# hall-lab/svtyper

Hardware: AMD Instinct MI355X
Metric: breakpoints genotyped/sec (higher is better)
Workload: dtype f64

## Files before the change

svtyper_amd/csrc/svt_batch_create.h:

```cpp

struct StageTimer {
    bool on = std::getenv("SVT_TRACE") != nullptr;
    std::chrono::steady_clock::time_point t0 = std::chrono::steady_clock::now();
    void mark(const char* what)
    {
        if (!on) return;
        const auto t1 = std::chrono::steady_clock::now();
        std::fprintf(stderr, "[svt] %-28s %8.2f ms\n", what, std::chrono::duration<double, std::milli>(t1 - t0).count());
        t0 = t1;
    }
};

int record_error(uint32_t err_bits)
{
    return fail(SVT_ERR_INVALID, record_error_text(err_bits));
}

int check_stream_errors(svt_batch* b)
{
    if (b->layout != kLayoutStream || !b->d_err) return SVT_OK;
    uint32_t bits = 0;
    HIP_TRY(hipMemcpyAsync(&bits, b->d_err, sizeof(uint32_t), hipMemcpyDeviceToHost, b->stream));
    HIP_TRY(hipStreamSynchronize(b->stream));
    return bits ? record_error(bits) : SVT_OK;
}

int ensure_result_slots(svt_batch* b, uint64_t slots)
{
    const uint64_t bytes = std::max<uint64_t>(slots, 1) * ((b->flags & SVT_FLAG_RESULT96) ? sizeof(svt_result96) : sizeof(svt_result));
    if (bytes <= b->cap_out) return SVT_OK;
    HIP_TRY(hipStreamSynchronize(b->stream));
    const bool bound = b->out_dev != b->d_out;
    g_pool.put(b->device, b->d_out, b->cap_out);
    b->d_out = nullptr;
    b->cap_out = 0;
    void* p = nullptr;
    SVT_TRY(g_pool.get(b->device, bytes, &p, &b->cap_out));
    b->d_out = static_cast<svt_result*>(p);
    if (!bound) {
        b->out_dev = b->d_out;
        b->sargs.out = b->d_out;
        b->pargs.out = b->d_out;
    }
    return SVT_OK;
}

uint64_t max_batch_records()
{
    static const uint64_t cached = [] {
        uint64_t v = 0xFFFFFFF0ull - 1;
        if (const char* e = std::getenv("SVT_MAX_BATCH_RECORDS")) {
            const uint64_t w = std::strtoull(e, nullptr, 10);
            if (w > 0 && w < v) v = w;
        }
        return v;
    }();
    return cached;
}

SmallRegion small_region(size_t tab, const size_t region_bytes, const bool l10_in_front, const size_t l10_bytes = 0, const uint32_t n_l10 = 0)
{
    SmallRegion r;
    if (l10_in_front && tab + l10_bytes + region_bytes <= (160 * 1024 / 2)) {
        r.l10_where = kL10Shared;
        r.lds_l10 = (uint32_t)tab;
        r.l10_entries = n_l10;
        tab += l10_bytes;
    }
    if (tab + region_bytes <= 160 * 1024) {
        r.region = (uint32_t)tab;
        r.lds_bytes = tab + region_bytes;
    }
    return r;
}

int create_stream(const svt_evidence_batch* in, svt_batch* b, void* d_records_resident = nullptr, uint64_t resident_cap = 0,
                  bool defer_records = false)
{
    const uint64_t n = in->n_units;
    const uint64_t n_rec = n ? in->rec_offset[n] : 0;
    StageTimer tm;
    if (n_rec > max_batch_records())
        return fail(SVT_ERR_INVALID, "too many records in one batch (< 2^32): cut it with svt_chunk_bounds, or hand it to svt_genotype, which does");
    uint64_t max_f = 0;
    bool wide_var_length = false, all_hinted = n > 0;
    {
        const uint64_t kChunk = 16384, n_chunks = (n + kChunk - 1) / kChunk;
        struct Part { uint64_t max_f = 0; int bad = 0; bool wide = false, hinted = true; };
        std::vector<Part> parts(std::max<uint64_t>(n_chunks, 1));
        parallel_for(n_chunks, [&](uint64_t ch) {
            Part p;
            for (uint64_t u = ch * kChunk; u < std::min(n, (ch + 1) * kChunk); ++u) {
                if (in->rec_offset[u + 1] < in->rec_offset[u]) { p.bad |= 1; continue; }
                const uint64_t f = in->rec_offset[u + 1] - in->rec_offset[u];
                if (f > 0x3FFFFFFFull) p.bad |= 2;
                const svt_unit& U = in->units[u];
                if (U.svtype > SVT_SVTYPE_BND) p.bad |= 4;
                if ((U.libs >> 24) != 0 || (U.flags & ~SVT_UNIT_SKIP)) p.bad |= 8;
                const uint32_t w_lo = SVT_UNIT_LIBS_FIRST(U.libs), w_cnt = SVT_UNIT_LIBS_COUNT(U.libs);
                if (w_cnt && w_lo + w_cnt > in->n_libs) p.bad |= 16;
                p.hinted = p.hinted && w_cnt != 0;
                if (U.var_length < -(1 << 30) || U.var_length > (1 << 30)) p.wide = true;
                p.max_f = std::max(p.max_f, f);
            }
            parts[ch] = p;
        });
        int bad = 0;
        for (uint64_t ch = 0; ch < n_chunks; ++ch) {
            bad |= parts[ch].bad;
            max_f = std::max(max_f, parts[ch].max_f);
            wide_var_length = wide_var_length || parts[ch].wide;
            all_hinted = all_hinted && parts[ch].hinted;
        }
        if (bad & 1) return fail(SVT_ERR_INVALID, "rec_offset not monotone");
        if (bad & 2) return fail(SVT_ERR_INVALID, "unit with too many records");
        if (bad & 4) return fail(SVT_ERR_INVALID, "bad svtype");
        if (bad & 8) return fail(SVT_ERR_INVALID, "unit reserved/flags bits must be 0");
        if (bad & 16) return fail(SVT_ERR_INVALID, "unit library window beyond n_libs");
    }
    tm.mark("validate units");
    HostTables T;
    SVT_TRY(build_tables(in, max_f, T));
    if (wide_var_length) T.fast_geometry = false;

    b->window_tiles = (SVT_STREAM_R == 1 && SVT_WINDOW_TILES == 2 && n >= kTwoTilesMinUnits) ? 2 : SVT_STREAM_R;
#ifndef SVT_WINDOW_SPLIT
#define SVT_WINDOW_SPLIT 0
#endif
    const bool split_kinds = SVT_WINDOW_SPLIT && b->window_tiles == 2 && !(b->flags & SVT_FLAG_SSO_ASSOCIATION) && !std::getenv("SVT_NO_WINDOW_SPLIT");
    auto window_budget_kernel = [&]() { return split_kinds ? window_kernel_of_kind(2) : stream_kernel_of(b, b->window_tiles); };
    const uint32_t kUnitsPerWg = (uint32_t)kBlock * (uint32_t)b->window_tiles;
    std::vector<uint32_t> perm;
    std::vector<uint2> chunks;
    std::vector<WgDesc> windows;
    struct Group { uint32_t begin, end; WgDesc w; };
    std::vector<Group> groups;
    uint32_t max_win_bins = 0, max_win_libs = 0;
    uint64_t all_bins = 0;
    for (const LibDesc& L : T.libs) all_bins += L.n_bins + 1;
    const bool whole_batch_window = !all_hinted && n > 0 && in->n_libs <= 255 &&
                                    kSBins + all_bins * 4 + in->n_libs * sizeof(WinLib) + 64 + kWavesPerBlock * kStreamRingBytes <= (160 * 1024 / 2);
    const uint32_t whole_key = SVT_UNIT_LIBS(0u, in->n_libs);
    const bool may_window = in->n_libs > 1 && T.fast_geometry && !(b->flags & SVT_FLAG_GENERAL_TABLES);
    bool windowed = may_window && (all_hinted || whole_batch_window);
    const bool derive_windows = may_window && !windowed && n > 0 && T.narrow_bins;
    if (derive_windows) defer_records = false;
    b->records_resident = !defer_records;
    auto group_units = [&](auto&& hint_of) -> bool {
        std::vector<uint32_t> start(65537, 0u);
        std::vector<uint16_t> count_of(65536, 0);
        for (uint64_t u = 0; u < n; ++u) {
            const uint32_t h = hint_of(u), first = SVT_UNIT_LIBS_FIRST(h), cnt = SVT_UNIT_LIBS_COUNT(h);
            if (cnt == 0) return false;
            count_of[first] = std::max(count_of[first], (uint16_t)cnt);
            ++start[first + 1];
        }
        for (uint32_t k = 0; k < 65536u; ++k) start[k + 1] += start[k];
        perm.resize(n);
        groups.clear();
        {
            std::vector<uint32_t> at(start.begin(), start.end() - 1);
            for (uint64_t u = 0; u < n; ++u) perm[at[SVT_UNIT_LIBS_FIRST(hint_of(u))]++] = (uint32_t)u;
        }
        for (uint32_t k = 0; k < 65536u; ++k) {
            if (start[k + 1] == start[k]) continue;
            const uint32_t lo = k, cnt = count_of[k];
            WgDesc w{};
            w.lib_lo = lo;
            w.lib_cnt = cnt;
            w.bin_lo = T.libs[lo].tab_off;
            w.bin_cnt = T.libs[lo + cnt - 1].tab_off + T.libs[lo + cnt - 1].n_bins + 1 - w.bin_lo;
            max_win_bins = std::max(max_win_bins, w.bin_cnt);
            max_win_libs = std::max(max_win_libs, w.lib_cnt);
            groups.push_back(Group{start[k], start[k + 1], w});
        }
        return true;
    };
    auto cut_chunks = [&](const uint32_t per_chunk) {
        chunks.clear();
        windows.clear();
        for (const Group& g : groups) {
            const uint32_t units = g.end - g.begin, pieces = (units + per_chunk - 1) / per_chunk;
            for (uint32_t i = 0; i < pieces; ++i) {
                const uint32_t p0 = g.begin + (uint32_t)((uint64_t)units * i / pieces), p1 = g.begin + (uint32_t)((uint64_t)units * (i + 1) / pieces);
                chunks.push_back(make_uint2(p0, p1 - p0));
                windows.push_back(g.w);
            }
        }
    };
    if (windowed) {
        windowed = group_units([&](uint64_t u) -> uint32_t { return all_hinted ? in->units[u].libs : whole_key; });
        tm.mark("group units by library window");
    }
    const uint32_t n_l10 = (uint32_t)T.l10.size();
    T.l10.resize(((size_t)n_l10 + 127) / 128 * 128, 0.0);
    tm.mark("build tables");

    SVT_TRY(g_handles.get_stream(&b->stream));
    SVT_TRY(g_handles.get_event(&b->ev0, true));
    SVT_TRY(g_handles.get_event(&b->ev1, true));

    const uint64_t n_blk = std::max<uint64_t>((n_rec + kBlockRecords - 1) / kBlockRecords, 1);
    {
        Stager st(b->stream);
        void* p = nullptr;
        if (d_records_resident) {
            if (resident_cap < n_blk * 128) return fail(SVT_ERR_INTERNAL, "resident record buffer too small");
            b->d_records = d_records_resident;
            b->cap_records = resident_cap;
        } else {
            SVT_TRY(g_pool.get(b->device, n_blk * 128, &p, &b->cap_records, true));
            b->d_records = p;
        }
        if (n_blk * 128 > n_rec * 16)
            HIP_TRY(hipMemsetAsync(static_cast<char*>(b->d_records) + n_rec * 16, 0, n_blk * 128 - n_rec * 16, b->stream));
        if (!d_records_resident && !defer_records) SVT_TRY(st.copy(b->d_records, in->records, n_rec * sizeof(uint4)));
        SVT_TRY(g_pool.get(b->device, (n + 1) * sizeof(uint64_t), &p, &b->cap_off));
        b->d_off = static_cast<uint64_t*>(p);
        if (n) SVT_TRY(st.copy(b->d_off, in->rec_offset, (n + 1) * sizeof(uint64_t)));
        SVT_TRY(g_pool.get(b->device, std::max<uint64_t>(n, 1) * sizeof(svt_unit), &p, &b->cap_units));
        b->d_units = static_cast<svt_unit*>(p);
        SVT_TRY(st.copy(b->d_units, in->units, n * sizeof(svt_unit)));
        SVT_TRY(upload(&b->d_libs, T.libs, st));
        SVT_TRY(upload(&b->d_pm, T.pm, st));
        SVT_TRY(upload(&b->d_l10, T.l10, st));
        SVT_TRY(upload(&b->d_bins, T.bins, st));
        SVT_TRY(upload(&b->d_wtab, T.wtab, st));
        SVT_TRY(g_pool.get(b->device, std::max<uint64_t>(n, 1) * sizeof(svt_result), &p, &b->cap_out));
        b->d_out = static_cast<svt_result*>(p);
        SVT_TRY(g_handles.get_small(sizeof(uint32_t), &p));
        b->d_err = static_cast<uint32_t*>(p);
        HIP_TRY(hipMemsetAsync(b->d_err, 0, sizeof(uint32_t), b->stream));
        SVT_TRY(st.finish());
    }
    tm.mark("H2D CSR + tables (staged)");

    if (derive_windows) {
        void* pp = nullptr;
        SVT_TRY(g_pool.get(b->device, n * sizeof(uint32_t), &pp, &b->cap_perm));
        b->d_perm = static_cast<uint32_t*>(pp);
        const uint32_t n32 = (uint32_t)n;
        const unsigned waves = (unsigned)std::min<uint64_t>(n, 256ull * 32);
        const dim3 grid((waves + kScanBlock / kWave - 1) / (kScanBlock / kWave)), block(kScanBlock);
        hipLaunchKernelGGL(svt_window_scan_kernel, grid, block, 0, b->stream, static_cast<const uint4*>(b->d_records), b->d_off, n32, b->d_perm);
        HIP_TRY(hipGetLastError());
        std::vector<uint32_t> seen(n);
        HIP_TRY(hipMemcpyAsync(seen.data(), b->d_perm, n * sizeof(uint32_t), hipMemcpyDeviceToHost, b->stream));
        HIP_TRY(hipStreamSynchronize(b->stream));
        tm.mark("library windows from the records (device scan)");
        bool all_seen = true;
        for (uint64_t u = 0; u < n && all_seen; ++u) all_seen = seen[u] != 0u && SVT_UNIT_LIBS_FIRST(seen[u]) + SVT_UNIT_LIBS_COUNT(seen[u]) <= in->n_libs;
        if (all_seen) {
            windowed = group_units([&](uint64_t u) -> uint32_t { return seen[u]; });
            tm.mark("group units by library window");
        }
    }

    size_t kStreamLdsPerWg = (160 * 1024 / 3) & ~size_t(127);
    constexpr size_t kStreamLdsPerWg2 = (160 * 1024 / 2) & ~size_t(127);
    constexpr size_t kLdsBin = 2 * sizeof(uint16_t);
    const size_t single_lds = kSBins + T.bins.size() * kLdsBin;
    const bool single = in->n_libs == 1 && T.fast_geometry && T.narrow_bins && single_lds + kWavesPerBlock * kStreamRingBytes <= 96 * 1024 &&
                        !(b->flags & SVT_FLAG_GENERAL_TABLES);
    const size_t window_lds = kSBins + (((size_t)max_win_bins * kLdsBin + 15) & ~size_t(15)) + (size_t)max_win_libs * sizeof(WinLib);
    windowed = windowed && T.narrow_bins && max_win_libs <= 32 && window_lds + kWavesPerBlock * kStreamRingBytes <= kStreamLdsPerWg2;
    b->mode = single ? kSingleLds : windowed ? kMultiLds : kGeneral;
    if (b->mode == kGeneral && in->n_libs > 1024)
        return fail(SVT_ERR_UNSUPPORTED, "more than 1024 libraries in a batch without usable library windows (svt_unit.libs)");
    bool identity = true;
    if (windowed) {
        uint32_t per_chunk = kUnitsPerWg;
        {
            int wgs = 3;
            hipFuncAttributes fa{};
            if (hipFuncGetAttributes(&fa, window_budget_kernel()) == hipSuccess && fa.numRegs > 0) wgs = std::max(1, std::min(8, 512 / ((fa.numRegs + 7) / 8 * 8)));
            else (void)hipGetLastError();
            const size_t lds = ((window_lds + 127) & ~size_t(127)) + kWavesPerBlock * kStreamRingBytes;
            const uint32_t resident = (uint32_t)std::min<size_t>((size_t)wgs, (160 * 1024) / lds) * cu_count(b->device);
            uint64_t n_min = 0;
            for (const Group& g : groups) n_min += (g.end - g.begin + kUnitsPerWg - 1) / kUnitsPerWg;
            per_chunk = balanced_units_per_wg(n, n_min, kUnitsPerWg, resident);
            if (per_chunk < kUnitsPerWg && resident) {
                const uint64_t rounds = (n_min + resident - 1) / resident;
                auto count = [&](uint32_t per) { uint64_t c = 0; for (const Group& g : groups) c += (g.end - g.begin + per - 1) / per; return c; };
                while (per_chunk < kUnitsPerWg && count(per_chunk) > rounds * resident) ++per_chunk;
            }
        }
        cut_chunks(per_chunk);
        Stager st(b->stream);
        void* pp = nullptr;
        for (uint64_t u = 0; u < n && identity; ++u) identity = perm[u] == (uint32_t)u;
        if (!identity) {
            if (!b->d_perm) {
                SVT_TRY(g_pool.get(b->device, std::max<uint64_t>(n, 1) * sizeof(uint32_t), &pp, &b->cap_perm));
                b->d_perm = static_cast<uint32_t*>(pp);
            }
            SVT_TRY(st.copy(b->d_perm, perm.data(), n * sizeof(uint32_t)));
        }
        SVT_TRY(upload(&b->d_chunks, chunks, st));
        SVT_TRY(upload(&b->d_windows, windows, st));
        SVT_TRY(st.finish());
        b->n_chunks = (uint32_t)chunks.size();
        uint32_t n_one = 0;
        while (n_one < b->n_chunks && windows[n_one].lib_cnt == 1u) ++n_one;
        bool ordered = true;
        for (uint32_t i = n_one; i < b->n_chunks && ordered; ++i) ordered = windows[i].lib_cnt != 1u;
        b->n_chunks_one = n_one;
        b->split_window_kinds = split_kinds && ordered;
    }
    if (b->d_perm && (!windowed || identity)) {
        g_pool.put(b->device, b->d_perm, b->cap_perm);
        b->d_perm = nullptr;
        b->cap_perm = 0;
    }
    StreamArgs& a = b->sargs;
    a.records = static_cast<const uint4*>(b->d_records);
    a.rec_offset = b->d_off;
    a.units = b->d_units;
    a.pm = b->d_pm;
    a.l10 = b->d_l10;
    a.libs = b->d_libs;
    a.bins = b->d_bins;
    a.wtab = b->d_wtab;
    a.n_l10 = n_l10;
    a.n_libs = in->n_libs;
    a.total_bins = (uint32_t)T.bins.size();
    a.last_blk = (uint32_t)(n_blk - 1);
    a.lds_bins = single ? a.total_bins : windowed ? max_win_bins : 0u;
    a.lds_libs = single || windowed ? 0u : in->n_libs;
    a.perm = b->d_perm;
    a.chunks = b->d_chunks;
    a.windows = b->d_windows;
    a.lds_winlibs = (uint32_t)(kSBins + (((size_t)a.lds_bins * kLdsBin + 15) & ~size_t(15)));
    size_t tables = a.lds_winlibs + (size_t)a.lds_libs * sizeof(LibDesc) + (windowed ? (size_t)max_win_libs * sizeof(WinLib) : 0);
    tables = (tables + 127) & ~size_t(127);
    if (single) {
        int wgs = 3;
        hipFuncAttributes fa{};
        if (hipFuncGetAttributes(&fa, stream_kernel_of(b, 1)) == hipSuccess && fa.numRegs > 0) wgs = std::max(1, std::min(8, 512 / ((fa.numRegs + 7) / 8 * 8)));
        else (void)hipGetLastError();
        const size_t by_lds = (160 * 1024) / (tables + kWavesPerBlock * kStreamRingBytes);
        b->one_tile_round_units = (uint64_t)std::min<size_t>((size_t)wgs, std::max<size_t>(by_lds, 1)) * cu_count(b->device) * kBlock;
    }
    {
        int wgs = 3;
        hipFuncAttributes fa{};
        if (hipFuncGetAttributes(&fa, b->mode == kMultiLds ? window_budget_kernel() : stream_kernel_of(b, tiles_per_wave(b, n))) == hipSuccess && fa.numRegs > 0)
            wgs = std::max(1, std::min(8, 512 / ((fa.numRegs + 7) / 8 * 8)));
        else
            (void)hipGetLastError();
        if (const char* e = std::getenv("SVT_STREAM_WGS_PER_CU")) wgs = std::max(1, std::atoi(e));
#ifdef SVT_FORCE_WGS
        wgs = SVT_FORCE_WGS;
#endif
        kStreamLdsPerWg = (160 * 1024 / (size_t)wgs) & ~size_t(127);
        b->wgs_per_cu = wgs;
    }
    const size_t l10_bytes = ((size_t)n_l10 * 8 + 127) & ~size_t(127);
    const size_t base_lds = tables + kWavesPerBlock * kStreamRingBytes;
    const size_t fit = std::max<size_t>(1, std::min<size_t>((size_t)b->wgs_per_cu, (160 * 1024) / base_lds));
    const size_t budget = ((160 * 1024) / fit) & ~size_t(127);
    (void)kStreamLdsPerWg;
    if (base_lds + l10_bytes <= budget) {
        a.l10_where = kL10Shared;
        a.lds_l10 = (uint32_t)tables;
        a.l10_lds_entries = n_l10;
        tables += l10_bytes;
    } else if (kStreamDepth == 1 && SVT_L10_THROUGH_RING) {
        a.l10_where = kL10Ring;
        a.l10_lds_entries = (uint32_t)std::min<uint64_t>((n_l10 + 127u) / 128u * 128u, kStreamRingBytes / 8);
    } else {
        a.l10_where = kL10Global;
        a.l10_lds_entries = 0;
    }
    a.lds_rings = (uint32_t)tables;
    if (b->mode == kSingleLds && a.l10_where != kL10Ring) {
        const size_t tab = (a.lds_winlibs + 127) & ~size_t(127);
        b->coop = small_region(tab, kCoopRegionBytes, true, l10_bytes, n_l10);
        if (b->coop.lds_bytes) {
            int wgs = 2;
            hipFuncAttributes fa{};
            if (hipFuncGetAttributes(&fa, coop_kernel_of(b)) == hipSuccess && fa.numRegs > 0) wgs = std::max(1, std::min(4, 512 / ((fa.numRegs + 7) / 8 * 8) * 4 / kCoopWaves));
            else (void)hipGetLastError();
            b->coop_resident = (uint32_t)std::min<size_t>((size_t)wgs, (160 * 1024) / b->coop.lds_bytes) * cu_count(b->device);
            if (b->coop.lds_bytes > 64 * 1024) HIP_TRY(hipFuncSetAttribute(coop_kernel_of(b), hipFuncAttributeMaxDynamicSharedMemorySize, (int)b->coop.lds_bytes));
        }
        b->split = small_region(tab, kSplitRegionBytes, true, l10_bytes, n_l10);
        if (b->split.lds_bytes > 64 * 1024)
            for (int lanes = 2; lanes <= 4; lanes += 2)
                HIP_TRY(hipFuncSetAttribute(split_kernel_of(b, lanes), hipFuncAttributeMaxDynamicSharedMemorySize, (int)b->split.lds_bytes));
    }
    if (b->mode == kMultiLds && a.l10_where != kL10Ring) {
        b->split = small_region((tables + 127) & ~size_t(127), kSplitRegionBytes, false);
        if (b->split.lds_bytes) {
            b->split.l10_where = a.l10_where;
            b->split.lds_l10 = a.lds_l10;
            b->split.l10_entries = a.l10_lds_entries;
        }
        if (b->split.lds_bytes > 64 * 1024)
            for (int lanes = 2; lanes <= 4; lanes += 2)
                if (lanes == 4 || !(b->flags & SVT_FLAG_SSO_ASSOCIATION))
                    HIP_TRY(hipFuncSetAttribute(split_kernel_of(b, lanes), hipFuncAttributeMaxDynamicSharedMemorySize, (int)b->split.lds_bytes));
    }
    a.n_units = n;
    a.unit_begin = 0;
    a.unit_end = (uint32_t)n;
    a.units_per_wg = (uint32_t)kBlock * (uint32_t)tiles_per_wave(b, n);
    a.result96 = (b->flags & SVT_FLAG_RESULT96) ? 1u : 0u;
    a.slot_begin = 0;
    b->resident_wgs = (uint32_t)std::min<size_t>((size_t)b->wgs_per_cu, (160 * 1024) / (tables + kWavesPerBlock * kStreamRingBytes)) *
                      cu_count(b->device);
    b->out_dev = b->d_out;
    b->out_slots = !a.result96 ? n : b->mode == kMultiLds ? (uint64_t)b->n_chunks * kBlock * (uint64_t)b->window_tiles : slots_of_launch(b, n);
    SVT_TRY(ensure_result_slots(b, b->out_slots));
    a.out = b->d_out;
    a.err = b->d_err;
    a.lib0 = T.libs[0];
    fill_gt_consts(a.c, in->split_weight, in->disc_weight);
    b->out_dev = b->d_out;
    b->lds_bytes = tables + kWavesPerBlock * kStreamRingBytes;
    if (b->lds_bytes > 160 * 1024) return fail(SVT_ERR_INVALID, "LDS budget exceeded");
    if (tm.on)
        std::fprintf(stderr, "[svt] kernel budget: %d workgroups/CU by registers, LDS %zu B/workgroup (%zu fit), log10 table (%u entries) %s (%u entries)\n",
                     b->wgs_per_cu, b->lds_bytes, (size_t)(160 * 1024) / std::max<size_t>(b->lds_bytes, 1), n_l10,
                     a.l10_where == kL10Shared ? "in LDS" : a.l10_where == kL10Ring ? "through the ring" : "through L2", a.l10_lds_entries);
    if (b->lds_bytes > 64 * 1024)
        for (int tiles = 1; tiles <= 2; ++tiles)
            if (b->mode != kGeneral || tiles == 1)
                HIP_TRY(hipFuncSetAttribute(stream_kernel_of(b, tiles), hipFuncAttributeMaxDynamicSharedMemorySize, (int)b->lds_bytes));
    if (b->lds_bytes > 64 * 1024 && b->split_window_kinds)
        for (int kind = 1; kind <= 2; ++kind)
            HIP_TRY(hipFuncSetAttribute(window_kernel_of_kind(kind), hipFuncAttributeMaxDynamicSharedMemorySize, (int)b->lds_bytes));
    return SVT_OK;
}
```

svtyper_amd/csrc/svt_batch_state.h:

```cpp


void free_batch(svt_batch* b)
{
    if (!b) return;
    (void)hipSetDevice(b->device);
    if (b->stream) (void)hipStreamSynchronize(b->stream);
    auto F = [](void* p) { g_handles.put_small(p); };
    g_pool.put(b->device, b->d_out, b->cap_out);
    g_pool.put(b->device, b->d_records, b->cap_records);
    g_pool.put(b->device, b->d_off, b->cap_off);
    g_pool.put(b->device, b->d_units, b->cap_units);
    g_pool.put(b->device, b->d_soff, b->cap_soff);
    g_pool.put(b->device, b->d_perm, b->cap_perm);
    F(b->d_chunks); F(b->d_windows);
    F(b->d_err);
    F(b->d_pm); F(b->d_l10); F(b->d_libs);
    F(b->d_bins); F(b->d_wtab);
    g_handles.put_event(b->ev0, true);
    g_handles.put_event(b->ev1, true);
    g_handles.put_stream(b->stream);
    delete b;
}

struct BatchFree {
    void operator()(svt_batch* b) const { free_batch(b); }
};
using BatchOwner = std::unique_ptr<svt_batch, BatchFree>;

int new_batch(BatchOwner* owner, int device, unsigned flags, int layout, uint64_t n_units, uint64_t n_records)
{
    owner->reset(new (std::nothrow) svt_batch());
    svt_batch* b = owner->get();
    if (!b) return fail(SVT_ERR_NOMEM, "out of host memory");
    b->device = device;
    b->flags = flags;
    b->layout = layout;
    b->n_units = n_units;
    b->n_records = n_records;
    return SVT_OK;
}

int check_device(int device)
{
    const int ndev = svt_device_count();
    if (ndev <= 0) return fail(SVT_ERR_NO_DEVICE, "no HIP device available (this library has no CPU fallback)");
    if (device < 0 || device >= ndev) return fail(SVT_ERR_NO_DEVICE, "device index out of range");
    return SVT_OK;
}

int select_device(int device)
{
    SVT_TRY(check_device(device));
    HIP_TRY(hipSetDevice(device));
    return SVT_OK;
}

const char* evidence_error(const svt_evidence_batch* in, unsigned flags, bool records_may_be_null = false)
{
    const uint64_t n = in->n_units;
    if (flags & ~kKnownFlags) return "unknown flag bits";
    if (n >= 0xFFFFFFF0ull) return "too many units in one batch (< 2^32)";
    if (in->n_libs == 0 || in->n_libs > 65536 || !in->libs) return "n_libs must be 1..65536";
    if (n && (!in->rec_offset || !in->units)) return "null unit arrays";
    if (n && in->rec_offset[0] != 0) return "rec_offset[0] must be 0";
    if (n && in->rec_offset[n] && !in->records && !records_may_be_null) return "null records";
    if (!(in->split_weight >= 0.0) || !(in->disc_weight >= 0.0) || !std::isfinite(in->split_weight) || !std::isfinite(in->disc_weight))
        return "weights must be finite and >= 0";
    return nullptr;
}

struct DevScratch {
    void* p = nullptr;
    ~DevScratch() { if (p) (void)hipFree(p); }
    int alloc(size_t bytes)
    {
        HIP_TRY(hipMalloc(&p, std::max<size_t>(bytes, 16)));
        return SVT_OK;
    }
    template <typename T> T* as() const { return static_cast<T*>(p); }
};

struct Pooled {
    int device;
    void* p = nullptr;
    uint64_t cap = 0;
    ~Pooled() { g_pool.put(device, p, cap); }
    int get(uint64_t bytes, bool records = false) { return g_pool.get(device, bytes, &p, &cap, records); }
    void* release() { void* q = p; p = nullptr; return q; }
};

struct CallStream {
    hipStream_t s = nullptr;
    ~CallStream() { if (s) g_handles.put_stream(s); }
    int take() { return g_handles.get_stream(&s); }
    void drain() { if (s) (void)hipStreamSynchronize(s); }
};

template <typename T>
int upload(T** dptr, const std::vector<T>& v, Stager& st)
{
    void* p = nullptr;
    const uint64_t bytes = std::max<size_t>(v.size(), 1) * sizeof(T);
    if (bytes <= (1u << 20)) SVT_TRY(g_handles.get_small(bytes, &p));
    else HIP_TRY(hipMalloc(&p, bytes));
    *dptr = static_cast<T*>(p);
    return st.copy(*dptr, v.data(), v.size() * sizeof(T));
}

template <typename T>
int upload(DevScratch& d, const std::vector<T>& v, Stager& st)
{
    SVT_TRY(d.alloc(v.size() * sizeof(T)));
    return st.copy(d.p, v.data(), v.size() * sizeof(T));
}

template <bool SSO>
const void* stream_kernel_for(int mode, int tiles)
{
    if (mode == kSingleLds && tiles == 2) return reinterpret_cast<const void*>(&svt_stream_kernel<SSO, kSingleLds, 2>);
    if (mode == kMultiLds && tiles == 2) return reinterpret_cast<const void*>(&svt_stream_kernel<SSO, kMultiLds, 2>);
    return mode == kSingleLds  ? reinterpret_cast<const void*>(&svt_stream_kernel<SSO, kSingleLds, SVT_STREAM_R>)
           : mode == kMultiLds ? reinterpret_cast<const void*>(&svt_stream_kernel<SSO, kMultiLds, SVT_STREAM_R>)
                               : reinterpret_cast<const void*>(&svt_stream_kernel<SSO, kGeneral, SVT_STREAM_R>);
}

const void* window_kernel_of_kind(int kind)
{
    return kind == 1 ? reinterpret_cast<const void*>(&svt_stream_kernel<false, kMultiLds, 2, 1>)
                     : reinterpret_cast<const void*>(&svt_stream_kernel<false, kMultiLds, 2, 2>);
}

const void* stream_kernel_of(const svt_batch* b, int tiles = SVT_STREAM_R)
{
    return (b->flags & SVT_FLAG_SSO_ASSOCIATION) ? stream_kernel_for<true>(b->mode, tiles) : stream_kernel_for<false>(b->mode, tiles);
}

const void* coop_kernel_of(const svt_batch* b)
{
    return (b->flags & SVT_FLAG_SSO_ASSOCIATION) ? reinterpret_cast<const void*>(&svt_coop_kernel<true, kSingleLds>)
                                                  : reinterpret_cast<const void*>(&svt_coop_kernel<false, kSingleLds>);
}

const void* split_kernel_of(const svt_batch* b, int lanes)
{
    const bool sso = (b->flags & SVT_FLAG_SSO_ASSOCIATION) != 0;
    if (b->mode == kMultiLds) {
        if (lanes == 2) return reinterpret_cast<const void*>(&svt_split_kernel<false, kMultiLds, 2>);
        return sso ? reinterpret_cast<const void*>(&svt_split_kernel<true, kMultiLds, 4>) : reinterpret_cast<const void*>(&svt_split_kernel<false, kMultiLds, 4>);
    }
    if (lanes == 2) return sso ? reinterpret_cast<const void*>(&svt_split_kernel<true, kSingleLds, 2>) : reinterpret_cast<const void*>(&svt_split_kernel<false, kSingleLds, 2>);
    return sso ? reinterpret_cast<const void*>(&svt_split_kernel<true, kSingleLds, 4>) : reinterpret_cast<const void*>(&svt_split_kernel<false, kSingleLds, 4>);
}

constexpr uint64_t kTwoTilesMinUnits = 768ull * kBlock * 9 / 8;
int tiles_per_wave(const svt_batch* b, uint64_t units)
{
#if SVT_STREAM_R == 1 && !defined(SVT_STREAM_ONE_TILE)
    if (b->mode == kSingleLds && units > (b->one_tile_round_units ? b->one_tile_round_units : kTwoTilesMinUnits)) return 2;
#endif
    (void)b; (void)units;
    return SVT_STREAM_R;
}

#ifndef SVT_L10_THROUGH_RING
#define SVT_L10_THROUGH_RING 0
#endif

inline uint32_t cu_count(int device)
{
    static std::mutex lock;
    static std::vector<int> known;
    std::lock_guard<std::mutex> g(lock);
    if ((size_t)device >= known.size()) known.resize((size_t)device + 1, 0);
    if (known[(size_t)device] == 0) {
        int v = 0;
        if (hipDeviceGetAttribute(&v, hipDeviceAttributeMultiprocessorCount, device) != hipSuccess || v <= 0) { (void)hipGetLastError(); v = 256; }
        known[(size_t)device] = v;
    }
    return (uint32_t)known[(size_t)device];
}

#ifndef SVT_WG_BALANCE
#define SVT_WG_BALANCE 1
#endif
#ifndef SVT_WG_MIN_FILL
#define SVT_WG_MIN_FILL 50
#endif
struct WgPlan { int tiles; uint32_t per_wg, n_wg; bool coop; int split; };
static std::atomic<int> g_wg_balance{SVT_WG_BALANCE && !std::getenv("SVT_NO_WG_BALANCE") ? SVT_WG_MIN_FILL : 0};
extern "C" int svt_debug_wg_balance(int min_fill_percent) { return g_wg_balance.exchange(std::max(0, std::min(100, min_fill_percent))); }
inline uint32_t balanced_units_per_wg(uint64_t units, uint64_t n_min, uint32_t full, uint32_t resident)
{
    const int min_fill = g_wg_balance.load(std::memory_order_relaxed);
    if (!min_fill || !resident || n_min <= resident) return full;
    const uint64_t rounds = (n_min + resident - 1) / resident;
    const uint64_t want = (units + rounds * resident - 1) / (rounds * resident);
    return want * 100 >= (uint64_t)full * (uint64_t)min_fill ? (uint32_t)want : full;
}
static std::atomic<uint32_t> g_force_per_wg{0}, g_force_tiles{0};
extern "C" void svt_debug_force_wg(uint32_t per_wg, uint32_t tiles) { g_force_per_wg = per_wg; g_force_tiles = tiles; }
#ifndef SVT_COOP_MAX_UNITS
#define SVT_COOP_MAX_UNITS (1ull << 40)
#endif
static std::atomic<uint64_t> g_coop_max_units{std::getenv("SVT_NO_COOP") ? uint64_t(0) : uint64_t(SVT_COOP_MAX_UNITS)};
static std::atomic<uint32_t> g_coop_per_wg{0};
extern "C" void svt_debug_coop(uint64_t max_units, uint32_t per_wg) { g_coop_max_units = max_units; g_coop_per_wg = per_wg; }
#ifndef SVT_SMALL_KIND
#define SVT_SMALL_KIND 0
#endif
#ifndef SVT_SPLIT4_CU_UNITS
#define SVT_SPLIT4_CU_UNITS 256
#endif
#ifndef SVT_SPLIT2_CU_UNITS
#define SVT_SPLIT2_CU_UNITS 512
#endif
#ifndef SVT_COOP_CU_UNITS
#define SVT_COOP_CU_UNITS 64
#endif
static std::atomic<int> g_small_kind{SVT_SMALL_KIND};
extern "C" int svt_debug_small_kind(int kind) { return g_small_kind.exchange(kind); }
int split_lanes_for(const svt_batch* b, uint64_t units)
{
    const int kind = g_small_kind.load(std::memory_order_relaxed);
    const bool sso = (b->flags & SVT_FLAG_SSO_ASSOCIATION) != 0;
    if (!b->split.lds_bytes || !units) return 0;
    if (kind == 3) return sso && b->mode == kMultiLds ? 0 : 2;
    if (kind == 4) return 4;
    if (kind != 0) return 0;
    const uint64_t cus = cu_count(b->device);
    const bool coop_first = b->coop.lds_bytes && units <= std::min<uint64_t>(cus * SVT_COOP_CU_UNITS, g_coop_max_units.load(std::memory_order_relaxed));
    if (coop_first) return 0;
    return units <= cus * SVT_SPLIT4_CU_UNITS ? 4 : units <= cus * SVT_SPLIT2_CU_UNITS && !sso ? 2 : 0;
}

WgPlan wg_plan(const svt_batch* b, uint64_t units)
{
    WgPlan p;
    p.coop = false;
    p.split = 0;
    {
        const int kind = g_small_kind.load(std::memory_order_relaxed);
        const int lanes = split_lanes_for(b, units);
        if (lanes && b->split.lds_bytes && units && !g_force_per_wg.load(std::memory_order_relaxed)) {
            p.split = lanes;
            p.tiles = 1;
            p.per_wg = (uint32_t)kBlock;
            p.n_wg = (uint32_t)((units + p.per_wg - 1) / p.per_wg);
            return p;
        }
        if (kind == 1 || kind == 3 || kind == 4) goto stream;
    }
    if (b->coop.lds_bytes && units && g_small_kind.load(std::memory_order_relaxed) != 1 &&
        (units <= std::min<uint64_t>((uint64_t)cu_count(b->device) * SVT_COOP_CU_UNITS, g_coop_max_units.load(std::memory_order_relaxed)) ||
         g_small_kind.load(std::memory_order_relaxed) == 2) &&
        !g_force_per_wg.load(std::memory_order_relaxed)) {
        p.coop = true;
        p.per_wg = (uint32_t)kBlock;
        if (const uint32_t f = g_coop_per_wg.load(std::memory_order_relaxed)) p.per_wg = std::min<uint32_t>((f + 63u) / 64u * 64u, (uint32_t)kBlock);
        else
            for (uint32_t per = 64; per < (uint32_t)kBlock; per += 64)
                if ((units + per - 1) / per <= std::max<uint32_t>(b->coop_resident, 1)) { p.per_wg = per; break; }
        p.tiles = (int)(p.per_wg / 64u);
        p.n_wg = (uint32_t)((units + p.per_wg - 1) / p.per_wg);
        return p;
    }
stream:
    if (const uint32_t f = g_force_per_wg.load(std::memory_order_relaxed)) {
        const int ft = (int)g_force_tiles.load(std::memory_order_relaxed);
        p.tiles = b->mode == kSingleLds && (ft == 1 || ft == 2) ? ft : tiles_per_wave(b, units);
        p.per_wg = std::min<uint32_t>(f, (uint32_t)kBlock * (uint32_t)p.tiles);
        p.n_wg = (uint32_t)((units + p.per_wg - 1) / p.per_wg);
        return p;
    }
    p.tiles = tiles_per_wave(b, units);
    const uint32_t full = (uint32_t)kBlock * (uint32_t)p.tiles;
    p.per_wg = balanced_units_per_wg(units, (units + full - 1) / full, full, b->resident_wgs);
    p.n_wg = (uint32_t)((units + p.per_wg - 1) / p.per_wg);
    return p;
}

uint64_t slots_of_launch(const svt_batch* b, uint64_t units)
{
    if (units == 0) return 0;
    if (b->layout == kLayoutPacked) return (units + kBlock - 1) / kBlock * kBlock;
    const WgPlan p = wg_plan(b, units);
    if (p.coop) return (uint64_t)p.n_wg * (uint64_t)p.tiles * (uint64_t)kWave;
    return (uint64_t)p.n_wg * (uint64_t)kBlock * (uint64_t)p.tiles;
}

int launch_stream(svt_batch* b, StreamArgs& a, hipStream_t stream)
{
    const uint64_t units = (uint64_t)a.unit_end - a.unit_begin;
    const WgPlan p = wg_plan(b, units);
    a.units_per_wg = p.per_wg;
    if (p.split) {
        StreamArgs c = a;
        b->split.apply(c);
        const dim3 grid(p.n_wg), block(kBlock * p.split);
        void* params[] = {&c};
        HIP_TRY(hipLaunchKernel(split_kernel_of(b, p.split), grid, block, params, b->split.lds_bytes, stream));
        return SVT_OK;
    }
    if (p.coop) {
        StreamArgs c = a;
        b->coop.apply(c);
        const dim3 grid(p.n_wg), block(kCoopBlock);
        void* params[] = {&c};
        HIP_TRY(hipLaunchKernel(coop_kernel_of(b), grid, block, params, b->coop.lds_bytes, stream));
        return SVT_OK;
    }
    const dim3 grid(p.n_wg), block(kBlock);
    void* params[] = {&a};
    HIP_TRY(hipLaunchKernel(stream_kernel_of(b, p.tiles), grid, block, params, b->lds_bytes, stream));
    return SVT_OK;
}

int packed_libs_mode(const uint32_t n_libs) { return n_libs <= 1 ? kOneLibrary : n_libs <= kShortSwitchLibs ? kLibsInLds : kLibsInHbm; }
const void* packed_kernel_of(const svt_batch* b)
{
    const bool sso = (b->flags & SVT_FLAG_SSO_ASSOCIATION) != 0;
    switch (packed_libs_mode(b->pargs.n_libs)) {
    case kOneLibrary: return sso ? reinterpret_cast<const void*>(&svt_packed_kernel<true, 1, kOneLibrary>) : reinterpret_cast<const void*>(&svt_packed_kernel<false, 1, kOneLibrary>);
    case kLibsInLds: return sso ? reinterpret_cast<const void*>(&svt_packed_kernel<true, 1, kLibsInLds>) : reinterpret_cast<const void*>(&svt_packed_kernel<false, 1, kLibsInLds>);
    default: return sso ? reinterpret_cast<const void*>(&svt_packed_kernel<true, 1, kLibsInHbm>) : reinterpret_cast<const void*>(&svt_packed_kernel<false, 1, kLibsInHbm>);
    }
}

int launch_range(svt_batch* b, uint64_t u0, uint64_t u1, hipStream_t stream, uint64_t slot_begin = 0)
{
    if (u1 <= u0) return SVT_OK;
    if (b->layout == kLayoutPacked) {
        PackedArgs a = b->pargs;
        a.unit_begin = (uint32_t)u0;
        a.unit_end = (uint32_t)u1;
        a.slot_begin = (uint32_t)slot_begin;
        const dim3 grid((unsigned)((u1 - u0 + kBlock - 1) / kBlock)), block(kBlock);
        void* params[] = {&a};
        HIP_TRY(hipLaunchKernel(packed_kernel_of(b), grid, block, params, b->lds_bytes, stream));
        return SVT_OK;
    }
    StreamArgs a = b->sargs;
    a.unit_begin = (uint32_t)u0;
    a.unit_end = (uint32_t)u1;
    a.slot_begin = (uint32_t)slot_begin;
    return launch_stream(b, a, stream);
}

int ensure_result_slots(svt_batch* b, uint64_t slots);

int launch_genotype(svt_batch* b)
{
    if (b->layout == kLayoutPacked) {
        if (b->n_units == 0) return SVT_OK;
        const dim3 grid((unsigned)((b->n_units + kBlock - 1) / kBlock)), block(kBlock);
        void* params[] = {&b->pargs};
        HIP_TRY(hipLaunchKernel(packed_kernel_of(b), grid, block, params, b->lds_bytes, b->stream));
        return SVT_OK;
    }
    if (b->n_units == 0) return SVT_OK;
    if (b->mode == kMultiLds && b->window_tiles == 1) {
        if (const int lanes = split_lanes_for(b, b->n_units)) {
            StreamArgs c = b->sargs;
            b->split.apply(c);
            c.chunk_begin = 0;
            const dim3 grid(b->n_chunks), block(kBlock * lanes);
            void* params[] = {&c};
            HIP_TRY(hipLaunchKernel(split_kernel_of(b, lanes), grid, block, params, b->split.lds_bytes, b->stream));
            return SVT_OK;
        }
    }
    if (b->mode == kMultiLds && b->split_window_kinds) {
        const dim3 block(kBlock);
        if (b->n_chunks_one) {
            StreamArgs a = b->sargs;
            a.chunk_begin = 0;
            void* params[] = {&a};
            HIP_TRY(hipLaunchKernel(window_kernel_of_kind(1), dim3(b->n_chunks_one), block, params, b->lds_bytes, b->stream));
        }
        if (b->n_chunks > b->n_chunks_one) {
            StreamArgs a = b->sargs;
            a.chunk_begin = b->n_chunks_one;
            void* params[] = {&a};
            HIP_TRY(hipLaunchKernel(window_kernel_of_kind(2), dim3(b->n_chunks - b->n_chunks_one), block, params, b->lds_bytes, b->stream));
        }
        return SVT_OK;
    }
    if (b->mode != kMultiLds) {
        if (b->sargs.result96) {
            const uint64_t need = slots_of_launch(b, b->n_units);
            if (need != b->out_slots) {
                if (b->out_dev != b->d_out) {
                    if (need > b->bound_slots) return fail(SVT_ERR_STATE, "the pass needs more result slots than the bound device buffer holds");
                } else {
                    SVT_TRY(ensure_result_slots(b, need));
                }
                b->out_slots = need;
            }
        }
        return launch_stream(b, b->sargs, b->stream);
    }
    const dim3 grid(b->n_chunks), block(kBlock);
    void* params[] = {&b->sargs};
    HIP_TRY(hipLaunchKernel(stream_kernel_of(b, b->window_tiles), grid, block, params, b->lds_bytes, b->stream));
    return SVT_OK;
}
```

svtyper_amd/csrc/svt_small_kernels.hip:

```cpp
#include <hip/hip_runtime.h>

#include <cstdint>

#include "../../include/svtyper_hip.h"

#include "svt_common.h"
#include "svt_device_types.h"
#include "svt_unit_math.h"
#include "svt_stream_kernel.h"
#include "svt_split_kernel.h"

namespace svt {
template __global__ void svt_stream_kernel<false, kSingleLds, 1>(const StreamArgs);
template __global__ void svt_stream_kernel<true, kSingleLds, 1>(const StreamArgs);
template __global__ void svt_stream_kernel<false, kMultiLds, 1>(const StreamArgs);
template __global__ void svt_stream_kernel<true, kMultiLds, 1>(const StreamArgs);
template __global__ void svt_split_kernel<false, kSingleLds, 2>(const StreamArgs);
template __global__ void svt_split_kernel<true, kSingleLds, 2>(const StreamArgs);
template __global__ void svt_split_kernel<false, kSingleLds, 4>(const StreamArgs);
template __global__ void svt_split_kernel<true, kSingleLds, 4>(const StreamArgs);
template __global__ void svt_split_kernel<false, kMultiLds, 2>(const StreamArgs);
template __global__ void svt_split_kernel<false, kMultiLds, 4>(const StreamArgs);
template __global__ void svt_split_kernel<true, kMultiLds, 4>(const StreamArgs);
}
```

svtyper_amd/csrc/svt_split_kernel.h:

```cpp
#ifndef SVT_SPLIT_KERNEL_H
#define SVT_SPLIT_KERNEL_H

#include "svt_stream_kernel.h"

namespace svt {

constexpr uint32_t kSplitTileAt = 0;
constexpr uint32_t kSplitUnitAt = kSplitTileAt + kBlock * 16u;
constexpr uint32_t kSplitGateAt = kSplitUnitAt + kBlock * 4u;
constexpr uint32_t kSplitTallyAt = kSplitGateAt + kBlock * 4u;
constexpr uint32_t kSplitRingAt = kSplitTallyAt + 5u * kBlock * 8u;
constexpr uint32_t kSplitRegionBytes = kSplitRingAt + (uint32_t)(kBlock / kWave) * kRingBytes;
static_assert(kSplitRingAt % 128u == 0u, "rings are line-aligned");

typedef __attribute__((address_space(3))) const u32x4 lds_cu32x4_s;

template <int SHIFT>
__device__ __forceinline__ uint32_t dpp_row_shift(const uint32_t v)
{
    constexpr int ctrl = SHIFT > 0 ? 0x110 + SHIFT : 0x100 - SHIFT;
    return (uint32_t)__builtin_amdgcn_update_dpp((int)v, (int)v, ctrl, 0xf, 0xf, false);
}
template <int SHIFT>
__device__ __forceinline__ double dpp_row_shift_f64(const double x)
{
    return __hiloint2double((int)dpp_row_shift<SHIFT>((uint32_t)__double2hiint(x)), (int)dpp_row_shift<SHIFT>((uint32_t)__double2loint(x)));
}

template <bool SSO>
struct SplitSums {
    double ref_seq, alt_seq, alt_clip, ref_span, alt_span;
    double l_ref_seq, l_alt_seq, l_alt_clip;
    template <int SHIFT>
    __device__ __forceinline__ SplitSums shifted() const
    {
        SplitSums t;
        t.ref_seq = dpp_row_shift_f64<SHIFT>(ref_seq);
        t.alt_seq = dpp_row_shift_f64<SHIFT>(alt_seq);
        t.alt_clip = dpp_row_shift_f64<SHIFT>(alt_clip);
        t.ref_span = dpp_row_shift_f64<SHIFT>(ref_span);
        t.alt_span = dpp_row_shift_f64<SHIFT>(alt_span);
        if (SSO) {
            t.l_ref_seq = dpp_row_shift_f64<SHIFT>(l_ref_seq);
            t.l_alt_seq = dpp_row_shift_f64<SHIFT>(l_alt_seq);
            t.l_alt_clip = dpp_row_shift_f64<SHIFT>(l_alt_clip);
        } else {
            t.l_ref_seq = t.l_alt_seq = t.l_alt_clip = 0.0;
        }
        return t;
    }
};

struct SplitAddends {
    double rs_a, rs_b, p_seq, p_clip, alt_w, ref_w;
    bool cont;
};

template <bool SSO, int MODE, int K>
__global__ __launch_bounds__(kBlock * K, 4) void svt_split_kernel(const StreamArgs a)
{
    static_assert(MODE == kSingleLds || MODE == kMultiLds, "one library, or library windows (svt_unit.libs)");
    static_assert(K == 2 || K == 4, "two or four lanes per unit");
    constexpr uint32_t kWaves = 4u * K, kThreads = kWaves * kWave, kUnitsPerWave = kWave / K, kRecs = kBlockRecords / K;
    constexpr uint32_t kWaveRing = kUnitsPerWave * 128u;
    extern __shared__ __attribute__((aligned(16))) unsigned char smem[];
    if ((uint32_t)(size_t)(__attribute__((address_space(3))) unsigned char*)smem != 0u) __builtin_trap();
    const uint32_t tid = threadIdx.x, lane = tid % kWave;
    const uint32_t wave = (uint32_t)__builtin_amdgcn_readfirstlane((int)(tid / kWave));
    unsigned char* region = smem + a.lds_rings;
    uint4* s_tile = reinterpret_cast<uint4*>(region + kSplitTileAt);
    uint32_t* s_unit = reinterpret_cast<uint32_t*>(region + kSplitUnitAt);
    uint32_t* s_gate = reinterpret_cast<uint32_t*>(region + kSplitGateAt);
    double* s_tally = reinterpret_cast<double*>(region + kSplitTallyAt);
    unsigned char* rings = region + kSplitRingAt;

    const WgUnits g = wg_units<MODE>(a, (uint32_t)kBlock);
    const uint32_t wg_base = g.wg_base, n_here = g.n_here, wg_index = g.wg_index;
    const WgDesc wd = g.wd;
    const bool sorter = tid < (uint32_t)kBlock;

    uint32_t beg = 0u, cnt = 0u, my_unit = kPadUnit;
    svt_unit U{};
    if (sorter && tid < n_here) {
        my_unit = wg_unit_at<MODE>(a, wg_base, tid);
        const uint64_t lo = a.rec_offset[my_unit], hi = a.rec_offset[my_unit + 1];
        beg = (uint32_t)lo;
        cnt = (uint32_t)(hi - lo);
        U = a.units[my_unit];
    }
    stage_tables<MODE, kThreads, false>(smem, a, wd, tid);
    for (uint32_t i = tid; i < 5u * kBlock; i += kThreads) s_tally[i] = 0.0;

    {
        uint32_t* s_hist = reinterpret_cast<uint32_t*>(rings);
        uint32_t* s_start = s_hist + (kMaxSortKey + 1);
        uint32_t* s_wsum = s_start + (kMaxSortKey + 1);
        const uint32_t nblk = cnt ? ((beg & 7u) + cnt + 7u) >> 3 : 0u;
        const uint32_t key = sorter && tid < n_here ? min(nblk + 1u, kMaxSortKey) : 0u;
        if (sorter) s_hist[tid] = 0u;
        __syncthreads();
        uint32_t rank = 0u;
        if (sorter) rank = atomicAdd(&s_hist[key], 1u);
        __syncthreads();
        uint32_t h = 0u, incl = 0u;
        if (sorter) {
            h = s_hist[kMaxSortKey - tid];
            incl = wave_inclusive_scan(h, lane);
            if (lane == kWave - 1) s_wsum[wave] = incl;
        }
        __syncthreads();
        if (sorter) {
            uint32_t before = 0;
#pragma unroll
            for (int w = 0; w < kWavesPerBlock; ++w) before += (uint32_t)w < wave ? s_wsum[w] : 0u;
            s_start[kMaxSortKey - tid] = before + incl - h;
        }
        __syncthreads();
        if (sorter) {
            const bool is_del = U.svtype == SVT_SVTYPE_DEL;
            const bool small_del = MODE == kSingleLds && is_del && ((double)U.pos_delta < a.lib0.sd2);
            const uint32_t flags = (small_del ? 0u : kTileFmask) | (is_del ? kTileDel16 : 0u) | ((uint32_t)U.svtype << kTileSvtypeShift) |
                                   ((uint32_t)U.flags << kTileUflagsShift);
            const uint32_t sub2 = is_del ? (uint32_t)U.var_length + (MODE == kSingleLds ? (uint32_t)a.lib0.key_min : 0u) : 0x80000000u;
            const uint32_t pos = s_start[key] + rank;
            s_tile[pos] = make_uint4(beg, cnt, sub2, flags);
            s_unit[pos] = my_unit;
            if (MODE == kMultiLds) {
                uint32_t gated = 0u;
                if (is_del)
                    for (uint32_t l = 0; l < wd.lib_cnt; ++l)
                        gated |= ((double)U.pos_delta < reinterpret_cast<const WinLib*>(smem + a.lds_winlibs)[l].sd2 ? 1u : 0u) << l;
                s_gate[pos] = gated;
            }
        }
        __syncthreads();
    }

    const uint32_t hh = lane % K, pos = wave * kUnitsPerWave + lane / K;
    const uint4 me = s_tile[pos];
    const uint32_t first_rec = me.x, n_rec = me.y;
    const uint32_t head = first_rec & 7u, last = head + n_rec;
    const uint32_t nblk = n_rec ? (last + 7u) >> 3 : 0u;
    uint32_t max_blk = nblk;
#pragma unroll
    for (int d = 1; d < kWave; d <<= 1) max_blk = max(max_blk, (uint32_t)__shfl_xor((int)max_blk, d, kWave));
    max_blk = (uint32_t)__builtin_amdgcn_readfirstlane((int)max_blk);
    uint32_t min_blk = nblk;
#pragma unroll
    for (int d = 1; d < kWave; d <<= 1) min_blk = min(min_blk, (uint32_t)__shfl_xor((int)min_blk, d, kWave));
    min_blk = (uint32_t)__builtin_amdgcn_readfirstlane((int)min_blk);
    StreamCtx sc;
    sc.fmask = me.w & kTileFmask;
    sc.kmin = (uint32_t)a.lib0.key_min;
    sc.nb = a.lib0.n_bins;
    sc.sub2 = me.z;
    sc.hist_at = kSBins + a.total_bins * 2u;
    sc.wt0 = kSWtab + (me.w & kTileDel16) * 8u;
    sc.wt1 = sc.wt0 + 8u * 8u;
    sc.wh0 = 0u;
    const uint32_t gated = MODE == kMultiLds ? s_gate[pos] : 0u;
    const bool is_del = (me.w & kTileDel16) != 0u;
    const uint32_t lib_last = wd.lib_cnt - 1u, winlibs_at = a.lds_winlibs;
    const uint32_t neutral_w = MODE == kMultiLds ? wd.lib_lo << SVT_REC_LIB_SHIFT : 0u;
    const uint32_t lib_key = MODE == kMultiLds && wd.lib_cnt == 1u ? wd.lib_lo << SVT_REC_LIB_SHIFT : 0u;

    unsigned char* ring = rings + wave * kWaveRing;
    const uint32_t ring_addr = (uint32_t)(size_t)(__attribute__((address_space(3))) unsigned char*)ring;
    const uint32_t o = lane >> 3, rr = lane & 7u;
    constexpr int kFetches = (int)kUnitsPerWave / 8;
    uint32_t src_first[kFetches], src_end[kFetches], src_base[kFetches];
#pragma unroll
    for (int i = 0; i < kFetches; ++i) {
        const uint32_t u = 8u * (uint32_t)i + o;
        const uint4 e = s_tile[wave * kUnitsPerWave + u];
        src_first[i] = e.x;
        src_end[i] = e.x + e.y;
        src_base[i] = (e.x & ~7u) + (rr ^ ((u >> 1) & 7u));
    }
    const char* rec_bytes = reinterpret_cast<const char*>(a.records);
    auto fetch = [&](const uint32_t k) {
        if (k >= 1u && k + 1u < min_blk) {
#pragma unroll
            for (int i = 0; i < kFetches; ++i) {
                const uint32_t rec = src_base[i] + k * kBlockRecords;
                __builtin_amdgcn_global_load_lds(rec_bytes + ((uint64_t)rec << 4), (lds_void_ptr)(ring + (uint32_t)i * 1024u), 16, 0, SVT_STREAM_AUX);
            }
            return;
        }
#pragma unroll
        for (int i = 0; i < kFetches; ++i) {
            const uint32_t rec = src_base[i] + k * kBlockRecords;
            if (rec >= src_first[i] && rec < src_end[i])
                __builtin_amdgcn_global_load_lds(rec_bytes + ((uint64_t)rec << 4), (lds_void_ptr)(ring + (uint32_t)i * 1024u), 16, 0, SVT_STREAM_AUX);
        }
    };
    const uint32_t uw = lane / K;
    uint32_t rd[kRecs];
#pragma unroll
    for (uint32_t j = 0; j < kRecs; ++j) rd[j] = ring_addr + uw * 128u + (((hh * kRecs + j) ^ ((uw >> 1) & 7u)) << 4);

    RecordCheck<MODE> check;
    SplitSums<SSO> run = {0.0, 0.0, 0.0, 0.0, 0.0, 0.0, 0.0, 0.0};
    if (max_blk) fetch(0u);
    for (uint32_t k = 0; k < max_blk; ++k) {
        u32x4 w[kRecs];
        asm volatile("s_waitcnt vmcnt(0)" ::: "memory");
#pragma unroll
        for (uint32_t j = 0; j < kRecs; ++j) w[j] = *reinterpret_cast<lds_cu32x4_s*>((size_t)rd[j]);
        asm volatile("s_waitcnt lgkmcnt(0)" ::: "memory");
        if (k + 1 < max_blk) fetch(k + 1);
        SplitAddends x[kRecs];
        bool any_cont = false;
#pragma unroll
        for (uint32_t j0 = 0; j0 < kRecs; j0 += 2u) {
            u32x4 wj[2];
            double pm_a[2], pm_b[2], s0[2], s1[2], c0[2], c1[2];
            int32_t thr1[2];
            uint32_t h2[2], f3[2];
#pragma unroll
            for (uint32_t q = 0; q < 2u; ++q) {
                const uint32_t j = j0 + q;
                const bool mine = k * kBlockRecords + hh * kRecs + j - head < n_rec;
                wj[q].x = mine ? w[j].x : 0u;
                wj[q].y = mine ? w[j].y : 0u;
                wj[q].z = mine ? w[j].z : 0u;
                wj[q].w = mine ? w[j].w : neutral_w;
                check.see(wj[q], lib_key);
                if (MODE == kMultiLds) {
                    const uint32_t rel = SVT_REC_LIB(wj[q].w) - wd.lib_lo;
                    check.window_lib(rel);
                    const uint32_t l = min(rel, lib_last);
                    const u32x4 d = *reinterpret_cast<lds_cu32x4_s*>((size_t)(winlibs_at + l * (uint32_t)sizeof(WinLib)));
                    f3[q] = ((gated >> l) & 1u) ? 0u : (wj[q].w & 7u);
                    const uint32_t sub2 = is_del ? sc.sub2 + d.x : 0x80000000u;
                    const uint32_t i1 = min(wj[q].x - d.x, d.y), i2 = min(wj[q].x - sub2, d.y);
                    thr1[q] = lds_i16(d.z + (i1 << 1));
                    h2[q] = lds_u16(d.w + (i2 << 1));
                } else {
                    f3[q] = wj[q].w & sc.fmask;
                    const uint32_t i1 = min(wj[q].x - sc.kmin, sc.nb), i2 = min(wj[q].x - sc.sub2, sc.nb);
                    thr1[q] = lds_i16(kSBins + (i1 << 1));
                    h2[q] = lds_u16(sc.hist_at + (i2 << 1));
                }
                pm_a[q] = lds_f64(kSPm + byte0_x8(wj[q].y));
                pm_b[q] = lds_f64(kSPm + byte1_x8(wj[q].y));
                x[j].rs_a = lds_f64(kSPm + byte2_x8(wj[q].y));
                x[j].rs_b = lds_f64(kSPm + byte3_x8(wj[q].y));
                s0[q] = lds_f64(kSPmHalf + byte0_x8(wj[q].z));
                s1[q] = lds_f64(kSPmHalf + byte1_x8(wj[q].z));
                c0[q] = lds_f64(kSPmHalf + byte2_x8(wj[q].z));
                c1[q] = lds_f64(kSPmHalf + byte3_x8(wj[q].z));
            }
            __builtin_amdgcn_sched_barrier(0);
            double w_alt[2], w_ref[2];
#pragma unroll
            for (uint32_t q = 0; q < 2u; ++q) {
                const bool p_conc = (int32_t)h2[q] <= thr1[q];
                const uint32_t wa = (p_conc ? sc.wt1 : sc.wt0) | (f3[q] << 3);
                w_alt[q] = lds_f64(wa);
                w_ref[q] = lds_f64(wa + kSWref);
            }
            __builtin_amdgcn_sched_barrier(0);
#pragma unroll
            for (uint32_t q = 0; q < 2u; ++q) {
                const uint32_t j = j0 + q;
                const double pp = pm_a[q] * pm_b[q];
                x[j].p_seq = s0[q] + s1[q];
                x[j].p_clip = c0[q] + c1[q];
                x[j].alt_w = pp * w_alt[q];
                x[j].ref_w = pp * w_ref[q];
                x[j].cont = SSO && (wj[q].w & SVT_REC_CONTINUATION) != 0u;
                any_cont = any_cont || x[j].cont;
            }
        }
        const bool has_cont = SSO && __any(any_cont);
#pragma unroll
        for (uint32_t p = 0; p < (uint32_t)K; ++p) {
            if (hh == p) {
#pragma unroll
                for (uint32_t j = 0; j < kRecs; ++j) {
                    if (!SSO) {
                        run.ref_seq = (run.ref_seq + x[j].rs_a) + x[j].rs_b;
                        run.alt_seq += x[j].p_seq;
                        run.alt_clip += x[j].p_clip;
                    } else if (!has_cont) {
                        run.ref_seq += run.l_ref_seq;
                        run.alt_seq += run.l_alt_seq;
                        run.alt_clip += run.l_alt_clip;
                        run.l_ref_seq = x[j].rs_a + x[j].rs_b;
                        run.l_alt_seq = x[j].p_seq;
                        run.l_alt_clip = x[j].p_clip;
                    } else {
                        const bool cont = x[j].cont;
                        run.ref_seq += cont ? 0.0 : run.l_ref_seq;
                        run.alt_seq += cont ? 0.0 : run.l_alt_seq;
                        run.alt_clip += cont ? 0.0 : run.l_alt_clip;
                        run.l_ref_seq = ((cont ? run.l_ref_seq : 0.0) + x[j].rs_a) + x[j].rs_b;
                        run.l_alt_seq = (cont ? run.l_alt_seq : 0.0) + x[j].p_seq;
                        run.l_alt_clip = (cont ? run.l_alt_clip : 0.0) + x[j].p_clip;
                    }
                    run.alt_span += x[j].alt_w;
                    run.ref_span += x[j].ref_w;
                }
            }
            run = p + 1u < (uint32_t)K ? run.template shifted<1>() : run.template shifted<-(K - 1)>();
        }
    }
    if (hh == 0u) {
        if (SSO) {
            run.ref_seq += run.l_ref_seq;
            run.alt_seq += run.l_alt_seq;
            run.alt_clip += run.l_alt_clip;
        }
        s_tally[pos] = run.ref_seq;
        s_tally[kBlock + pos] = run.alt_seq;
        s_tally[2 * kBlock + pos] = run.alt_clip;
        s_tally[3 * kBlock + pos] = run.ref_span;
        s_tally[4 * kBlock + pos] = run.alt_span;
    }
    asm volatile("s_waitcnt vmcnt(0)" ::: "memory");
    __syncthreads();

    if (wave < (uint32_t)kWavesPerBlock) {
        const uint32_t p = wave * kWave + lane;
        Acc acc = {s_tally[p], s_tally[kBlock + p], s_tally[2 * kBlock + p], s_tally[3 * kBlock + p], s_tally[4 * kBlock + p], 0.0, 0.0, 0.0};
        const uint32_t unit = s_unit[p], flags = s_tile[p].w;
        const double* lds_l10 = reinterpret_cast<const double*>(smem + a.lds_l10);
        uint4 piece[8];
        unit_epilogue(acc, (flags >> kTileSvtypeShift) & 0xffu, flags >> kTileUflagsShift, a.c, lds_l10, a.l10, a.l10_where == kL10Shared ? a.l10_lds_entries : 0u, piece);
        uint32_t unit_out = unit;
        if (a.out_samples > 1u && unit != kPadUnit) {
            const uint32_t sample = unit / a.out_sites;
            unit_out = (unit - sample * a.out_sites) * a.out_samples + sample;
        }
        uint32_t tile_slot = 0xFFFFFFFFu;
        if (a.result96) {
            piece[5] = make_uint4(piece[5].x, piece[7].y, unit_out, 0u);
            tile_slot = a.slot_begin + (wg_index * (uint32_t)kWavesPerBlock + wave) * kWave;
        }
        store_result_records_through_ring(rings + wave * kRingBytes, piece, unit_out, lane, reinterpret_cast<unsigned char*>(a.out), a.result96 ? 6u : 8u, tile_slot);
    }
    const uint32_t bad = check.bits(MODE == kMultiLds ? wd.lib_cnt : a.n_libs);
    if (bad) atomicOr(a.err, bad);
}

}

#endif
```

svtyper_amd/csrc/svt_stream_kernel.h:

```cpp
#ifndef SVT_STREAM_KERNEL_H
#define SVT_STREAM_KERNEL_H

#ifndef SVT_STREAM_AUX
#define SVT_STREAM_AUX 2
#endif
#ifndef SVT_STREAM_EDGE_AUX
#define SVT_STREAM_EDGE_AUX 0
#endif
#ifndef SVT_STREAM_SPLIT
#define SVT_STREAM_SPLIT 4
#endif
#ifndef SVT_STREAM_WAVES
#define SVT_STREAM_WAVES 3
#endif
#ifndef SVT_WINDOW_WAVES
#define SVT_WINDOW_WAVES 3
#endif

#include <type_traits>

#include "svt_wg_parts.h"

namespace svt {

template <int MODE>
struct RecordCheck {
    uint32_t flags_or = 0, span_or = 0, lone = 0, lib_max = 0;
    __device__ __forceinline__ void see(const u32x4 w, const uint32_t lib_key = 0u)
    {
        if (MODE == kMultiLds) flags_or |= w.w ^ lib_key;
        else flags_or |= w.w;
        span_or |= w.x;
        lone = max(lone, (w.w & 0x17u) ^ 0x10u);
        if (MODE == kGeneral) lib_max = max(lib_max, w.w & 0xffff00u);
    }
    __device__ __forceinline__ void window_lib(const uint32_t d) { lib_max = max(lib_max, d); }
    __device__ __forceinline__ uint32_t bits(const uint32_t limit) const
    {
        const uint32_t n_libs = limit;
        const bool bad_lib = MODE == kSingleLds ? (flags_or & 0xffff00u) != 0u
                             : MODE == kMultiLds ? (limit == 1u ? (flags_or & 0xffff00u) != 0u : lib_max >= limit)
                                                 : (lib_max >> SVT_REC_LIB_SHIFT) >= n_libs;
        return (lone > 0x10u ? kErrStraddleNoPair : 0u) | (bad_lib ? kErrLibIndex : 0u) |
               ((flags_or & ~SVT_REC_FLAG_MASK) ? kErrReservedBits : 0u) | ((int32_t)span_or < 0 ? kErrNegativeSpan : 0u);
    }
};

template <bool SSO, bool EDGE, bool CONT = true>
__device__ __forceinline__ double record_weights(const u32x4 w, const bool mine, Acc& a)
{
    const uint32_t wy = EDGE ? (mine ? w.y : 0u) : w.y;
    const uint32_t wz = EDGE ? (mine ? w.z : 0u) : w.z;
    const double pm_a = lds_f64(kSPm + byte0_x8(wy)), pm_b = lds_f64(kSPm + byte1_x8(wy));
    const double rs_a = lds_f64(kSPm + byte2_x8(wy)), rs_b = lds_f64(kSPm + byte3_x8(wy));
    const double p_seq = lds_f64(kSPmHalf + byte0_x8(wz)) + lds_f64(kSPmHalf + byte1_x8(wz));
    const double p_clip = lds_f64(kSPmHalf + byte2_x8(wz)) + lds_f64(kSPmHalf + byte3_x8(wz));
    if (SSO && !CONT) {
        a.ref_seq += a.l_ref_seq;
        a.alt_seq += a.l_alt_seq;
        a.alt_clip += a.l_alt_clip;
        a.l_ref_seq = rs_a + rs_b;
        a.l_alt_seq = p_seq;
        a.l_alt_clip = p_clip;
    } else if (SSO) {
        const bool cont = (w.w & SVT_REC_CONTINUATION) != 0u;
        a.ref_seq += cont ? 0.0 : a.l_ref_seq;
        a.alt_seq += cont ? 0.0 : a.l_alt_seq;
        a.alt_clip += cont ? 0.0 : a.l_alt_clip;
        a.l_ref_seq = ((cont ? a.l_ref_seq : 0.0) + rs_a) + rs_b;
        a.l_alt_seq = (cont ? a.l_alt_seq : 0.0) + p_seq;
        a.l_alt_clip = (cont ? a.l_alt_clip : 0.0) + p_clip;
    } else {
        a.ref_seq = (a.ref_seq + rs_a) + rs_b;
        a.alt_seq += p_seq;
        a.alt_clip += p_clip;
    }
    return pm_a * pm_b;
}

template <bool SSO, bool EDGE, bool CONT>
__device__ __forceinline__ void record_single(const u32x4 w, const bool mine, const StreamCtx& c, Acc& a)
{
    const double pp = record_weights<SSO, EDGE, CONT>(w, mine, a);
    const uint32_t i1 = min(w.x - c.kmin, c.nb), i2 = min(w.x - c.sub2, c.nb);
    const int32_t thr1 = lds_i16(kSBins + (i1 << 1));
    const uint32_t h2 = lds_u16(c.hist_at + (i2 << 1));
    const bool p_conc = (int32_t)h2 <= thr1;
    const uint32_t wa = (p_conc ? c.wt1 : c.wt0) | ((w.w & c.fmask) << 3);
    a.alt_span += pp * lds_f64(wa);
    a.ref_span += pp * lds_f64(wa + kSWref);
}

struct WindowCtx {
    uint32_t lib_lo;
    uint32_t lib_last;
    uint32_t winlibs_at;
    uint32_t vl_or_never;
    uint32_t wt0, wt1;
    uint32_t wh0;
    uint32_t gated;
    bool is_del;
};

typedef __attribute__((address_space(3))) const u32x4 lds_cu32x4;

template <bool SSO, bool EDGE, bool CONT, class CHECK>
__device__ __forceinline__ void record_window(const u32x4 w, const bool mine, const WindowCtx& c, Acc& a, CHECK& check)
{
    const double pp = record_weights<SSO, EDGE, CONT>(w, mine, a);
    check.window_lib(EDGE && !mine ? 0u : SVT_REC_LIB(w.w) - c.lib_lo);
    const uint32_t la = c.winlibs_at + min(SVT_REC_LIB(w.w) - c.lib_lo, c.lib_last) * (uint32_t)sizeof(WinLib);
    const u32x4 d = *reinterpret_cast<lds_cu32x4*>((size_t)la);
    const uint32_t open = (uint32_t)__builtin_amdgcn_sbfe((int32_t)c.gated, min(SVT_REC_LIB(w.w) - c.lib_lo, c.lib_last), 1u);
    const uint32_t f3 = w.w & 7u & open;
    const uint32_t sub2 = c.vl_or_never + d.x;
    const uint32_t i1 = min(w.x - d.x, d.y), i2 = min(w.x - sub2, d.y);
    const int32_t thr1 = lds_i16(d.z + (i1 << 1));
    const uint32_t h2 = lds_u16(d.w + (i2 << 1));
    const bool p_conc = (int32_t)h2 <= thr1;
    const uint32_t wa = (p_conc ? c.wt1 : c.wt0) | (f3 << 3);
    a.alt_span += pp * lds_f64(wa);
    a.ref_span += pp * lds_f64(wa + kSWref);
}

template <bool SSO, int MODE, int R, int WK = 0>
__global__ __launch_bounds__(kBlock, MODE == kSingleLds ? SVT_STREAM_WAVES : MODE == kMultiLds ? (WK ? 4 : SVT_WINDOW_WAVES) : 2) void svt_stream_kernel(const StreamArgs a)
{
    static_assert(WK == 0 || (MODE == kMultiLds && !SSO), "window kinds: classic library-window kernels only");
    extern __shared__ __attribute__((aligned(16))) unsigned char smem[];
    constexpr uint32_t kUnitsPerWg = kBlock * R;
    if (MODE != kGeneral && (uint32_t)(size_t)(__attribute__((address_space(3))) unsigned char*)smem != 0u) __builtin_trap();
    unsigned char* rings = smem + a.lds_rings;
    const uint32_t tid = threadIdx.x, lane = tid % kWave;
    const uint32_t wave = (uint32_t)__builtin_amdgcn_readfirstlane((int)(tid / kWave));
    const WgUnits g = wg_units<MODE>(a);
    const uint32_t wg_base = g.wg_base, n_here = g.n_here, wg_index = g.wg_index;
    const WgDesc wd = g.wd;
    auto unit_at = [&](const uint32_t local) -> uint32_t { return wg_unit_at<MODE>(a, wg_base, local); };

    uint32_t beg[R], cnt[R];
#pragma unroll
    for (int j = 0; j < R; ++j) {
        const uint32_t local = (uint32_t)j * kBlock + tid;
        beg[j] = 0u;
        cnt[j] = 0u;
        if (local < n_here) {
            const uint32_t u = unit_at(local);
            const uint64_t lo = a.rec_offset[u], hi = a.rec_offset[u + 1];
            beg[j] = (uint32_t)lo;
            cnt[j] = (uint32_t)(hi - lo);
        }
    }

    stage_tables<MODE, kBlock, true>(smem, a, wd, tid);
    uint4 info[R];
    wg_sort_into_tiles<R>(rings, beg, cnt, n_here, tid, lane, wave, info);

    Tables t;
    t.pm = reinterpret_cast<double*>(smem + kSPm);
    t.wtab = reinterpret_cast<PairWeights*>(smem + kSWtab);
    t.libs = reinterpret_cast<LibDesc*>(smem + kSBins);
    t.bins = a.bins;

    unsigned char* ring = rings + wave * kStreamRingBytes;
    const uint32_t ring_addr = (uint32_t)(size_t)(__attribute__((address_space(3))) unsigned char*)ring;
    const uint32_t o = lane >> 3, rr = lane & 7u;
    const uint32_t col_even = (rr ^ (o >> 1)) << 4, col_odd = col_even ^ 64u;
    const uint32_t sw = (lane >> 1) & 7u;
    const uint32_t lane_block = ring_addr + lane * 128u, sw16 = sw << 4;
    const char* rec_bytes = reinterpret_cast<const char*>(a.records);

    RecordCheck<MODE> check;
    const uint32_t lib_key = MODE == kMultiLds && wd.lib_cnt == 1u ? wd.lib_lo << SVT_REC_LIB_SHIFT : 0u;

#pragma unroll
    for (int r = 0; r < R; ++r) {
        const uint32_t first_rec = info[r].x, n_rec = info[r].y;
        const uint32_t unit = info[r].z == kPadUnit ? kPadUnit : unit_at(info[r].z);
        svt_unit U{};
        if (unit != kPadUnit) U = a.units[unit];
        const uint32_t head = first_rec & 7u, last = head + n_rec;
        const uint32_t nblk = n_rec ? (last + 7u) >> 3 : 0u;
        uint32_t max_blk, min_blk;
        tile_block_range(nblk, max_blk, min_blk);
        uint32_t src_first[8], src_end[8], src_base[8];
#pragma unroll
        for (int i = 0; i < 8; ++i) {
            src_first[i] = (uint32_t)__shfl((int)first_rec, 8 * i + (int)o, kWave);
            src_end[i] = src_first[i] + (uint32_t)__shfl((int)n_rec, 8 * i + (int)o, kWave);
            src_base[i] = (src_first[i] & ~7u) + (((i & 1) ? col_odd : col_even) >> 4);
        }

        constexpr int kEdgeAux = R >= 2 ? SVT_STREAM_EDGE_AUX : SVT_STREAM_AUX;
        auto fetch_first = [&]() {
            fetch_block<kEdgeAux, true>(0, src_base, src_first, src_end, rec_bytes, ring);
        };
        auto fetch = [&](const uint32_t k, const uint32_t st = 0u) -> bool {
            unsigned char* stage = ring + st * kStageBytes;
            if (k + 1 < min_blk) {
                fetch_block_interior<SVT_STREAM_AUX>(k, src_base, rec_bytes, stage);
                return true;
            } else if (kEdgeAux != SVT_STREAM_AUX && k + 1 >= min_blk) {
                constexpr bool kLastUseInLastTile = R >= 2;
                if (kLastUseInLastTile && r == R - 1) fetch_block_tail_exact<SVT_STREAM_AUX, SVT_STREAM_AUX>(k, src_base, src_end, rec_bytes, stage);
                else fetch_block_tail_exact<SVT_STREAM_AUX, kEdgeAux>(k, src_base, src_end, rec_bytes, stage);
            } else
                fetch_block<SVT_STREAM_AUX, false>(k, src_base, src_first, src_end, rec_bytes, stage);
            return false;
        };

        LaneCtx c{};
        c.is_del = U.svtype == SVT_SVTYPE_DEL;
        c.del16 = c.is_del ? 16u : 0u;
        c.var_length = U.var_length;
        c.pos_delta_d = (double)U.pos_delta;
        StreamCtx sc;
        {
            const bool small_del = c.is_del && (c.pos_delta_d < a.lib0.sd2);
            sc.fmask = small_del ? 0u : 7u;
            sc.kmin = (uint32_t)a.lib0.key_min;
            sc.nb = a.lib0.n_bins;
            sc.sub2 = c.is_del ? (uint32_t)U.var_length + (uint32_t)a.lib0.key_min : 0x80000000u;
            sc.hist_at = kSBins + a.total_bins * 2u;
            sc.wt0 = kSWtab + c.del16 * 8u;
            sc.wt1 = sc.wt0 + 8u * 8u;
            sc.wh0 = kSWhi + c.del16 * 4u;
        }
        if (MODE == kMultiLds) {
            const WinLib w0 = reinterpret_cast<const WinLib*>(smem + a.lds_winlibs)[0];
            const bool small_del = c.is_del && (c.pos_delta_d < w0.sd2);
            sc.fmask = small_del ? 0u : 7u;
            sc.kmin = w0.kmin;
            sc.nb = w0.nb;
            sc.sub2 = c.is_del ? (uint32_t)U.var_length + w0.kmin : 0x80000000u;
            sc.hist_at = w0.hist_at;
        }
        WindowCtx wc;
        wc.lib_lo = wd.lib_lo;
        wc.lib_last = wd.lib_cnt - 1u;
        wc.winlibs_at = a.lds_winlibs;
        wc.vl_or_never = c.is_del ? (uint32_t)U.var_length : 0x80000000u;
        wc.wt0 = sc.wt0;
        wc.wt1 = sc.wt1;
        wc.wh0 = sc.wh0;
        wc.is_del = c.is_del;
        wc.gated = 0u;
        if (MODE == kMultiLds && c.is_del) {
            for (uint32_t l = 0; l < wd.lib_cnt; ++l)
                wc.gated |= (c.pos_delta_d < reinterpret_cast<const WinLib*>(smem + a.lds_winlibs)[l].sd2 ? 1u : 0u) << l;
        }
        wc.gated = ~wc.gated;
        Acc acc = {0.0, 0.0, 0.0, 0.0, 0.0, 0.0, 0.0, 0.0};

        auto consume = [&](const u32x4 (&w)[8], const uint32_t k, auto edge, auto window_kind, auto continuations) {
            constexpr bool EDGE = decltype(edge)::value;
            constexpr bool CONT = decltype(continuations)::value;
            constexpr int KIND = decltype(window_kind)::value;
            auto is_mine = [&](const int j) -> bool {
                const uint32_t idx = k * kBlockRecords + (uint32_t)j;
                return !EDGE || (idx >= head && idx < last);
            };
#pragma unroll
            for (int j = 0; j < 8; ++j) {
                if (j == SVT_STREAM_SPLIT) __builtin_amdgcn_sched_barrier(0);
                const bool mine = is_mine(j);
                const u32x4 wj = w[j];
                if (mine) check.see(wj, lib_key);
                if (MODE == kSingleLds) {
                    record_single<SSO, EDGE, CONT>(wj, mine, sc, acc);
                } else if (MODE == kMultiLds) {
                    if (KIND == 1) record_single<SSO, EDGE, CONT>(wj, mine, sc, acc);
                    else record_window<SSO, EDGE, CONT>(wj, mine, wc, acc, check);
                } else {
                    const uint32_t wy = mine ? wj.y : 0u, wz = mine ? wj.z : 0u;
                    weight_evidence<SSO>(wy >> 16 | (wz << 16), wz >> 16, (wj.w & SVT_REC_CONTINUATION) != 0, t, acc);
                    pair_evidence(wj.x, wy & 0xffffu, wj.w & 7u, min(SVT_REC_LIB(wj.w), a.n_libs - 1u), t, c, acc);
                }
            }
        };

        auto l10_into_ring = [&]() {
            const char* l10_bytes = reinterpret_cast<const char*>(a.l10);
            for (uint32_t off = 0; off < a.l10_lds_entries * 8u; off += 1024u)
                __builtin_amdgcn_global_load_lds(l10_bytes + off + lane * 16u, (lds_void_ptr)(ring + off), 16, 0, 0);
        };
        if (max_blk) {
            fetch_first();
            u32x4 w[8];
            bool exact_behind = false;
            if (kStreamDepth == 2 && max_blk > 1) exact_behind = fetch(1, 1);
#pragma unroll 1
            for (uint32_t k = 0; k < max_blk; ++k) {
                const uint32_t stage_off = kStreamDepth == 2 ? (k & 1u) * kStageBytes : 0u;
                if (kStreamDepth == 2) {
                    const bool pend = k + 1 < max_blk && exact_behind;
                    if (k & 1u) {
                        if (pend) read_block<kStageBytes, 8>(lane_block, sw16, w);
                        else read_block<kStageBytes, 0>(lane_block, sw16, w);
                    } else {
                        if (pend) read_block<0, 8>(lane_block, sw16, w);
                        else read_block<0, 0>(lane_block, sw16, w);
                    }
                } else {
                    read_block(lane_block, sw16, w);
                }
                auto refill = [&]() {
                    if (kStreamDepth == 2) {
                        if (k + 2 < max_blk) exact_behind = fetch(k + 2, k & 1u);
                    } else if (k + 1 < max_blk) fetch(k + 1);
                    else if (a.l10_where == kL10Ring) l10_into_ring();
                };
                const uint32_t k8 = k * kBlockRecords;
                const uint32_t neutral_w = MODE == kMultiLds ? wd.lib_lo << SVT_REC_LIB_SHIFT : 0u;
                if (__any(k8 < head || k8 + kBlockRecords > last)) {
#pragma unroll
                    for (int j = 0; j < 8; ++j) {
                        const bool mine = k8 + (uint32_t)j - head < n_rec;
                        w[j].x = mine ? w[j].x : 0u;
                        w[j].y = mine ? w[j].y : 0u;
                        w[j].z = mine ? w[j].z : 0u;
                        w[j].w = mine ? w[j].w : neutral_w;
                    }
                }
                bool has_cont = false;
                if (SSO && MODE != kGeneral)
                    has_cont = __any(((w[0].w | w[1].w | w[2].w | w[3].w | w[4].w | w[5].w | w[6].w | w[7].w) & SVT_REC_CONTINUATION) != 0u);
                if (SSO && MODE != kGeneral && has_cont) {
#pragma unroll 1
                    for (uint32_t j = 0; j < 8u; ++j) {
                        u32x4 wj = *reinterpret_cast<lds_cu32x4*>((size_t)(lane_block + stage_off + ((j << 4) ^ sw16)));
                        const bool mine = k8 + j - head < n_rec;
                        wj.x = mine ? wj.x : 0u;
                        wj.y = mine ? wj.y : 0u;
                        wj.z = mine ? wj.z : 0u;
                        wj.w = mine ? wj.w : neutral_w;
                        check.see(wj, lib_key);
                        if (MODE == kSingleLds || WK == 1 || (WK == 0 && !SSO && wd.lib_cnt == 1u)) record_single<SSO, false, true>(wj, true, sc, acc);
                        else record_window<SSO, false, true>(wj, true, wc, acc, check);
                    }
                    refill();
                    continue;
                }
                refill();
                using kind_any = std::integral_constant<int, 0>;
                using kind_one = std::integral_constant<int, 1>;
                auto run = [&](auto edge_tag, auto kind_tag) {
                    if (!SSO || MODE == kGeneral || has_cont) consume(w, k, edge_tag, kind_tag, std::true_type{});
                    else consume(w, k, edge_tag, kind_tag, std::false_type{});
                };
                if (MODE == kMultiLds && WK != 2 && (WK == 1 || (!SSO && wd.lib_cnt == 1u))) run(std::false_type{}, kind_one{});
                else run(std::false_type{}, kind_any{});
            }
        }
        if (SSO) {
            acc.ref_seq += acc.l_ref_seq;
            acc.alt_seq += acc.l_alt_seq;
            acc.alt_clip += acc.l_alt_clip;
        }

        const double* lds_l10 = reinterpret_cast<const double*>(a.l10_where == kL10Shared ? smem + a.lds_l10 : ring);
        if (a.l10_where == kL10Ring) {
            if (!max_blk || kStreamDepth == 2) l10_into_ring();
            asm volatile("s_waitcnt vmcnt(0)" ::: "memory");
        }
        uint4 piece[8];
        unit_epilogue(acc, (uint32_t)U.svtype, (uint32_t)U.flags, a.c, lds_l10, a.l10, a.l10_lds_entries, piece);

        uint32_t unit_out = unit;
        if (a.out_samples > 1u && unit != kPadUnit) {
            const uint32_t sample = unit / a.out_sites;
            unit_out = (unit - sample * a.out_sites) * a.out_samples + sample;
        }
        uint32_t tile_slot = 0xFFFFFFFFu;
        if (a.result96) {
            result96_tag(piece, unit_out);
            tile_slot = a.slot_begin + wg_index * kUnitsPerWg + ((uint32_t)r * kWavesPerBlock + ((r & 1) ? (uint32_t)kWavesPerBlock - 1u - wave : wave)) * kWave;
        }
        store_result_records_through_ring(ring, piece, unit_out, lane, reinterpret_cast<unsigned char*>(a.out), a.result96 ? 6u : 8u, tile_slot);
    }
    const uint32_t bad = check.bits(MODE == kMultiLds ? wd.lib_cnt : a.n_libs);
    if (bad) atomicOr(a.err, bad);
}

}

#endif
```

svtyper_amd/csrc/svt_wg_parts.h:

```cpp
#ifndef SVT_WG_PARTS_H
#define SVT_WG_PARTS_H

#include "svt_ring_engine.h"

namespace svt {

constexpr uint32_t kSPm = 0;
constexpr uint32_t kSPmHalf = kSPm + 256 * 8;
constexpr uint32_t kSWtab = kSPmHalf + 256 * 8;
constexpr uint32_t kSWref = 32 * 8;
constexpr uint32_t kSWhi = kSWtab + 2 * 32 * 8;
constexpr uint32_t kSWhiRef = 32 * 4;
constexpr uint32_t kSBins = kSWhi + 2 * 32 * 4;

struct StreamArgs {
    const uint4* records;
    const uint64_t* rec_offset;
    const svt_unit* units;
    const double* pm;
    const double* l10;
    const LibDesc* libs;
    const Bin* bins;
    const PairWeights* wtab;
    uint32_t n_l10;
    uint32_t n_libs;
    uint32_t total_bins;
    uint32_t last_blk;
    uint32_t lds_bins;
    uint32_t lds_libs;
    uint32_t lds_rings;
    uint32_t l10_where;
    uint32_t lds_l10;
    uint32_t l10_lds_entries;
    uint64_t n_units;
    svt_result* out;
    uint32_t* err;
    const uint32_t* perm;
    const uint2* chunks;
    const WgDesc* windows;
    uint32_t lds_winlibs;
    uint32_t unit_begin;
    uint32_t unit_end;
    uint32_t units_per_wg;
    uint32_t chunk_begin;
    uint32_t result96;
    uint32_t slot_begin;
    uint32_t out_samples;
    uint32_t out_sites;
    LibDesc lib0;
    GtConsts c;
};

struct WinLib {
    uint32_t kmin;
    uint32_t nb;
    uint32_t thr_at;
    uint32_t hist_at;
    double sd2;
    double pad;
};
static_assert(sizeof(WinLib) == 32, "WinLib is read as two 16-byte halves");

struct WgUnits {
    uint32_t wg_index;
    uint32_t wg_base;
    uint32_t n_here;
    WgDesc wd;
};
template <int MODE>
__device__ __forceinline__ WgUnits wg_units(const StreamArgs& a, const uint32_t chunk_cap = 0xFFFFFFFFu)
{
    WgUnits g;
    g.wg_base = a.unit_begin + blockIdx.x * a.units_per_wg;
    g.wd = WgDesc{};
    g.wg_index = MODE == kMultiLds ? blockIdx.x + a.chunk_begin : blockIdx.x;
    if (MODE == kMultiLds) {
        const uint2 ch = a.chunks[g.wg_index];
        g.wg_base = ch.x;
        g.n_here = min(ch.y, chunk_cap);
        g.wd = a.windows[g.wg_index];
    } else {
        g.n_here = min(a.units_per_wg, a.unit_end - g.wg_base);
    }
    return g;
}
template <int MODE>
__device__ __forceinline__ uint32_t wg_unit_at(const StreamArgs& a, const uint32_t wg_base, const uint32_t local)
{
    return MODE == kMultiLds && a.perm ? a.perm[wg_base + local] : wg_base + local;
}

template <int MODE, uint32_t THREADS, bool HI>
__device__ __forceinline__ void stage_tables(unsigned char* smem, const StreamArgs& a, const WgDesc& wd, const uint32_t tid)
{
    for (uint32_t i = tid; i < 256; i += THREADS) {
        const double p = a.pm[i];
        reinterpret_cast<double*>(smem + kSPm)[i] = p;
        reinterpret_cast<double*>(smem + kSPmHalf)[i] = p * 0.5;
    }
    if (tid < 32) {
        const PairWeights pw = a.wtab[tid];
        if (MODE != kGeneral) {
            reinterpret_cast<double*>(smem + kSWtab)[tid] = pw.w_alt;
            reinterpret_cast<double*>(smem + kSWtab + kSWref)[tid] = pw.w_ref;
            if (HI) {
                reinterpret_cast<uint32_t*>(smem + kSWhi)[tid] = (uint32_t)__double2hiint(pw.w_alt);
                reinterpret_cast<uint32_t*>(smem + kSWhi + kSWhiRef)[tid] = (uint32_t)__double2hiint(pw.w_ref);
            }
        } else {
            reinterpret_cast<PairWeights*>(smem + kSWtab)[tid] = pw;
        }
    }
    if (MODE == kSingleLds) {
        int16_t* s_thr = reinterpret_cast<int16_t*>(smem + kSBins);
        uint16_t* s_hst = reinterpret_cast<uint16_t*>(smem + kSBins) + a.total_bins;
        for (uint32_t i = tid; i < a.total_bins; i += THREADS) {
            const Bin bn = a.bins[i];
            s_thr[i] = (int16_t)bn.thr;
            s_hst[i] = (uint16_t)bn.hist;
        }
    } else if (MODE == kMultiLds) {
        int16_t* s_thr = reinterpret_cast<int16_t*>(smem + kSBins);
        uint16_t* s_hst = reinterpret_cast<uint16_t*>(smem + kSBins) + wd.bin_cnt;
        for (uint32_t i = tid; i < wd.bin_cnt; i += THREADS) {
            const Bin bn = a.bins[wd.bin_lo + i];
            s_thr[i] = (int16_t)bn.thr;
            s_hst[i] = (uint16_t)bn.hist;
        }
        if (tid < wd.lib_cnt) {
            const LibDesc L = a.libs[wd.lib_lo + tid];
            WinLib wl;
            wl.kmin = (uint32_t)L.key_min;
            wl.nb = L.n_bins;
            wl.thr_at = kSBins + (L.tab_off - wd.bin_lo) * 2u;
            wl.hist_at = kSBins + (wd.bin_cnt + L.tab_off - wd.bin_lo) * 2u;
            wl.sd2 = L.sd2;
            wl.pad = 0.0;
            reinterpret_cast<WinLib*>(smem + a.lds_winlibs)[tid] = wl;
        }
    } else {
        for (uint32_t i = tid; i < a.n_libs * (uint32_t)(sizeof(LibDesc) / 8); i += THREADS)
            reinterpret_cast<uint64_t*>(smem + kSBins)[i] = reinterpret_cast<const uint64_t*>(a.libs)[i];
    }
    if (a.l10_where == kL10Shared) {
        double* s_l10 = reinterpret_cast<double*>(smem + a.lds_l10);
        for (uint32_t i = tid; i < a.n_l10; i += THREADS) s_l10[i] = a.l10[i];
    }
}

struct StreamCtx {
    uint32_t fmask;
    uint32_t kmin;
    uint32_t nb;
    uint32_t sub2;
    uint32_t hist_at;
    uint32_t wt0, wt1;
    uint32_t wh0;
};

constexpr uint32_t kTileFmask = 7u, kTileDel16 = 16u, kTileSvtypeShift = 8u, kTileUflagsShift = 16u;
template <int MODE>
__device__ __forceinline__ uint4 make_tile_entry(const svt_unit& U, const uint32_t beg, const uint32_t cnt, const StreamArgs& a)
{
    const bool is_del = U.svtype == SVT_SVTYPE_DEL;
    const bool small_del = MODE == kSingleLds && is_del && ((double)U.pos_delta < a.lib0.sd2);
    const uint32_t flags = (small_del ? 0u : kTileFmask) | (is_del ? kTileDel16 : 0u) | ((uint32_t)U.svtype << kTileSvtypeShift) |
                           ((uint32_t)U.flags << kTileUflagsShift);
    const uint32_t sub2 = is_del ? (uint32_t)U.var_length + (MODE == kSingleLds ? (uint32_t)a.lib0.key_min : 0u) : 0x80000000u;
    return make_uint4(beg, cnt, sub2, flags);
}
__device__ __forceinline__ uint32_t tile_svtype(const uint32_t flags) { return (flags >> kTileSvtypeShift) & 0xffu; }
__device__ __forceinline__ uint32_t tile_uflags(const uint32_t flags) { return flags >> kTileUflagsShift; }

__device__ __forceinline__ uint32_t result_destination(const StreamArgs& a, const uint32_t unit)
{
    uint32_t unit_out = unit;
    if (a.out_samples > 1u && unit != kPadUnit) {
        const uint32_t sample = unit / a.out_sites;
        unit_out = (unit - sample * a.out_sites) * a.out_samples + sample;
    }
    return unit_out;
}
__device__ __forceinline__ void tally_epilogue(const StreamArgs& a, const unsigned char* smem, const double* s_tally, const uint4* s_tile,
                                               const uint32_t* s_unit, const uint32_t p, unsigned char* ring, const uint32_t lane,
                                               const uint32_t tile_slot)
{
    Acc acc = {s_tally[p], s_tally[kBlock + p], s_tally[2 * kBlock + p], s_tally[3 * kBlock + p], s_tally[4 * kBlock + p], 0.0, 0.0, 0.0};
    const uint32_t unit = s_unit[p], flags = s_tile[p].w;
    const double* lds_l10 = reinterpret_cast<const double*>(smem + a.lds_l10);
    uint4 piece[8];
    unit_epilogue(acc, tile_svtype(flags), tile_uflags(flags), a.c, lds_l10, a.l10, a.l10_where == kL10Shared ? a.l10_lds_entries : 0u, piece);
    const uint32_t unit_out = result_destination(a, unit);
    uint32_t sorted_base = 0xFFFFFFFFu;
    if (a.result96) {
        result96_tag(piece, unit_out);
        sorted_base = tile_slot;
    }
    store_result_records_through_ring(ring, piece, unit_out, lane, reinterpret_cast<unsigned char*>(a.out), a.result96 ? 6u : 8u, sorted_base);
}

}

#endif
```

svtyper_amd/csrc/svtyper_hip.hip:

```cpp

#include <hip/hip_runtime.h>

#include <algorithm>
#include <chrono>
#include <cmath>
#include <cstdint>
#include <cstdio>
#include <cstdlib>
#include <cstring>
#include <memory>
#include <mutex>
#include <string>
#include <thread>
#include <vector>

#include "../../include/svtyper_hip.h"
#include "../../include/svtyper_reads.h"

#ifndef SVT_WINDOW_TILES
#define SVT_WINDOW_TILES 2
#endif
#ifndef SVT_STREAM_R
#define SVT_STREAM_R 1
#endif

#include "svt_common.h"
#include "svt_device_types.h"
#include "svt_unit_math.h"
#include "svt_entry_formats.h"
#include "svt_pack.h"
#include "svt_stream_kernel.h"
#include "svt_packed_kernel.h"
#include "svt_coop_kernel.h"
#include "svt_split_kernel.h"
#include "svt_window_scan_kernel.h"
#include "svt_geometry_kernel.h"
#include "svt_evidence_kernel.h"
#include "svt_inflate_kernel.h"
#include "svt_crc32_kernel.h"
#include "svt_bgzf.h"
#include "svt_evidence_arena.h"
#include "svt_library_kernel.h"
#include "svt_library_arena.h"
#include "svt_bayes_kernel.h"
#include "svt_host_tables.h"
#include "svt_host_transfer.h"

using namespace svt;

#if SVT_STREAM_R == 1 && !defined(SVT_NO_SMALL_TU)
namespace svt {
extern template __global__ void svt_stream_kernel<false, kSingleLds, 1>(const StreamArgs);
extern template __global__ void svt_stream_kernel<true, kSingleLds, 1>(const StreamArgs);
extern template __global__ void svt_stream_kernel<false, kMultiLds, 1>(const StreamArgs);
extern template __global__ void svt_stream_kernel<true, kMultiLds, 1>(const StreamArgs);
extern template __global__ void svt_split_kernel<false, kSingleLds, 2>(const StreamArgs);
extern template __global__ void svt_split_kernel<true, kSingleLds, 2>(const StreamArgs);
extern template __global__ void svt_split_kernel<false, kSingleLds, 4>(const StreamArgs);
extern template __global__ void svt_split_kernel<true, kSingleLds, 4>(const StreamArgs);
extern template __global__ void svt_split_kernel<false, kMultiLds, 2>(const StreamArgs);
extern template __global__ void svt_split_kernel<false, kMultiLds, 4>(const StreamArgs);
extern template __global__ void svt_split_kernel<true, kMultiLds, 4>(const StreamArgs);
}
#endif

constexpr unsigned kKnownFlags = SVT_FLAG_SSO_ASSOCIATION | SVT_FLAG_GENERAL_TABLES | SVT_FLAG_RESULT96;

struct SmallRegion {
    size_t lds_bytes = 0;
    uint32_t region = 0, l10_where = kL10Global, lds_l10 = 0, l10_entries = 0;
    void apply(StreamArgs& a) const
    {
        a.lds_rings = region;
        a.l10_where = l10_where;
        a.lds_l10 = lds_l10;
        a.l10_lds_entries = l10_entries;
    }
};

struct svt_batch {
    int device = 0;
    unsigned flags = 0;
    hipStream_t stream = nullptr;
    uint64_t n_units = 0, n_records = 0;
    int mode = kSingleLds;
    int layout = kLayoutStream;
    size_t lds_bytes = 0;
    bool have_results = false;
    uint64_t cap_out = 0;
    double* d_pm = nullptr;
    double* d_l10 = nullptr;
    LibDesc* d_libs = nullptr;
    Bin* d_bins = nullptr;
    PairWeights* d_wtab = nullptr;
    svt_result* d_out = nullptr;
    svt_result* out_dev = nullptr;
    void* d_records = nullptr;
    uint64_t* d_off = nullptr;
    svt_unit* d_units = nullptr;
    uint64_t cap_records = 0, cap_off = 0, cap_units = 0;
    uint32_t* d_err = nullptr;
    uint32_t* d_perm = nullptr;
    uint2* d_chunks = nullptr;
    WgDesc* d_windows = nullptr;
    uint64_t cap_perm = 0;
    uint32_t n_chunks = 0;
    uint32_t n_chunks_one = 0;
    bool split_window_kinds = false;
    int window_tiles = 1;
    uint64_t bound_slots = 0;
    uint64_t out_slots = 0;
    bool records_resident = true;
    int wgs_per_cu = 3;
    uint32_t resident_wgs = 0;
    uint64_t one_tile_round_units = 0;
    SmallRegion coop, split;
    uint32_t coop_resident = 0;
    StreamArgs sargs{};
    uint32_t* d_soff = nullptr;
    uint64_t cap_soff = 0, n_slots = 0;
    PackedArgs pargs{};
    hipEvent_t ev0 = nullptr, ev1 = nullptr;
};

namespace {

#include "svt_batch_state.h"
#include "svt_batch_create.h"
#include "svt_batch_packed.h"
#include "svt_batch_oneshot.h"

}

extern "C" {

#include "svt_entry_batch.h"
#include "svt_entry_seams.h"
#include "svt_entry_packed.h"

void* svt_batch_stream(svt_batch* b) { return b ? (void*)b->stream : nullptr; }

void svt_batch_destroy(svt_batch* b) { free_batch(b); }

#include "svt_entry_debug.h"
#include "svt_entry_inflate.h"
#include "svt_entry_evidence.h"
#include "svt_entry_library.h"
#include "svt_entry_oneshot.h"

}
```

Measured before the change: 3.443 billion.

## Stage library-window tables over a shared bin space in LDS

Adds a shared bin-space layout for multi-library windows. Every library in a window gets a row of threshold and histogram entries indexed by a common key range, so the per-record lookup is a row multiply plus a clamped offset instead of going through per-library descriptors. Only the sd2 gates are kept, as a small double array. It is enabled only when the padded table fits and does not reduce workgroups per CU, and it disables window-kind splitting. The cost is more LDS for libraries with mismatched key ranges, plus extra kernel instantiations.

```diff
diff --git a/svtyper_amd/csrc/svt_batch_create.h b/svtyper_amd/csrc/svt_batch_create.h
--- a/svtyper_amd/csrc/svt_batch_create.h
+++ b/svtyper_amd/csrc/svt_batch_create.h
@@ -128,14 +128,15 @@
 #define SVT_WINDOW_SPLIT 0
 #endif
     const bool split_kinds = SVT_WINDOW_SPLIT && b->window_tiles == 2 && !(b->flags & SVT_FLAG_SSO_ASSOCIATION) && !std::getenv("SVT_NO_WINDOW_SPLIT");
-    auto window_budget_kernel = [&]() { return split_kinds ? window_kernel_of_kind(2) : stream_kernel_of(b, b->window_tiles); };
+    auto window_budget_kernel = [&]() { return split_kinds && !b->binspace ? window_kernel_of_kind(2) : stream_kernel_of(b, b->window_tiles); };
     const uint32_t kUnitsPerWg = (uint32_t)kBlock * (uint32_t)b->window_tiles;
     std::vector<uint32_t> perm;
     std::vector<uint2> chunks;
     std::vector<WgDesc> windows;
-    struct Group { uint32_t begin, end; WgDesc w; };
+    struct Group { uint32_t begin, end; WgDesc w; BinSpace bs; };
     std::vector<Group> groups;
     uint32_t max_win_bins = 0, max_win_libs = 0;
+    uint64_t max_binspace_bytes = 0;
     uint64_t all_bins = 0;
     for (const LibDesc& L : T.libs) all_bins += L.n_bins + 1;
     const bool whole_batch_window = !all_hinted && n > 0 && in->n_libs <= 255 &&
@@ -172,7 +173,9 @@
             w.bin_cnt = T.libs[lo + cnt - 1].tab_off + T.libs[lo + cnt - 1].n_bins + 1 - w.bin_lo;
             max_win_bins = std::max(max_win_bins, w.bin_cnt);
             max_win_libs = std::max(max_win_libs, w.lib_cnt);
-            groups.push_back(Group{start[k], start[k + 1], w});
+            const BinSpace bs = binspace_of(&T.libs[lo].key_min, &T.libs[lo].n_bins, cnt, (uint32_t)(sizeof(LibDesc) / sizeof(uint32_t)));
+            max_binspace_bytes = std::max(max_binspace_bytes, binspace_table_bytes(cnt, bs.nb));
+            groups.push_back(Group{start[k], start[k + 1], w, bs});
         }
         return true;
     };
@@ -265,6 +268,18 @@
     const size_t window_lds = kSBins + (((size_t)max_win_bins * kLdsBin + 15) & ~size_t(15)) + (size_t)max_win_libs * sizeof(WinLib);
     windowed = windowed && T.narrow_bins && max_win_libs <= 32 && window_lds + kWavesPerBlock * kStreamRingBytes <= kStreamLdsPerWg2;
     b->mode = single ? kSingleLds : windowed ? kMultiLds : kGeneral;
+    const size_t binspace_lds = kSBins + (((size_t)max_binspace_bytes + 15) & ~size_t(15)) + (size_t)max_win_libs * sizeof(double);
+    {
+        const size_t rings = kWavesPerBlock * kStreamRingBytes;
+        auto per_cu = [&](size_t tab) { return std::min<size_t>(4, (160 * 1024) / (((tab + 127) & ~size_t(127)) + rings)); };
+        b->binspace = windowed && max_binspace_bytes <= kStreamLdsPerWg2 && binspace_lds + rings <= kStreamLdsPerWg2 &&
+                      per_cu(binspace_lds) >= per_cu(window_lds) && !std::getenv("SVT_NO_WINDOW_BINSPACE");
+    }
+    if (b->binspace)
+        for (Group& g : groups) {
+            g.w.bin_lo = (uint32_t)g.bs.k0;
+            g.w.bin_cnt = g.bs.nb;
+        }
     if (b->mode == kGeneral && in->n_libs > 1024)
         return fail(SVT_ERR_UNSUPPORTED, "more than 1024 libraries in a batch without usable library windows (svt_unit.libs)");
     bool identity = true;
@@ -275,7 +290,7 @@
             hipFuncAttributes fa{};
             if (hipFuncGetAttributes(&fa, window_budget_kernel()) == hipSuccess && fa.numRegs > 0) wgs = std::max(1, std::min(8, 512 / ((fa.numRegs + 7) / 8 * 8)));
             else (void)hipGetLastError();
-            const size_t lds = ((window_lds + 127) & ~size_t(127)) + kWavesPerBlock * kStreamRingBytes;
+            const size_t lds = (((b->binspace ? binspace_lds : window_lds) + 127) & ~size_t(127)) + kWavesPerBlock * kStreamRingBytes;
             const uint32_t resident = (uint32_t)std::min<size_t>((size_t)wgs, (160 * 1024) / lds) * cu_count(b->device);
             uint64_t n_min = 0;
             for (const Group& g : groups) n_min += (g.end - g.begin + kUnitsPerWg - 1) / kUnitsPerWg;
@@ -306,7 +321,7 @@
         bool ordered = true;
         for (uint32_t i = n_one; i < b->n_chunks && ordered; ++i) ordered = windows[i].lib_cnt != 1u;
         b->n_chunks_one = n_one;
-        b->split_window_kinds = split_kinds && ordered;
+        b->split_window_kinds = split_kinds && ordered && !b->binspace;
     }
     if (b->d_perm && (!windowed || identity)) {
         g_pool.put(b->device, b->d_perm, b->cap_perm);
@@ -332,7 +347,9 @@
     a.chunks = b->d_chunks;
     a.windows = b->d_windows;
     a.lds_winlibs = (uint32_t)(kSBins + (((size_t)a.lds_bins * kLdsBin + 15) & ~size_t(15)));
-    size_t tables = a.lds_winlibs + (size_t)a.lds_libs * sizeof(LibDesc) + (windowed ? (size_t)max_win_libs * sizeof(WinLib) : 0);
+    if (b->binspace) a.lds_winlibs = (uint32_t)(binspace_lds - (size_t)max_win_libs * sizeof(double));
+    size_t tables = a.lds_winlibs + (size_t)a.lds_libs * sizeof(LibDesc) +
+                    (b->binspace ? (size_t)max_win_libs * sizeof(double) : windowed ? (size_t)max_win_libs * sizeof(WinLib) : 0);
     tables = (tables + 127) & ~size_t(127);
     if (single) {
         int wgs = 3;
@@ -424,6 +441,9 @@
         std::fprintf(stderr, "[svt] kernel budget: %d workgroups/CU by registers, LDS %zu B/workgroup (%zu fit), log10 table (%u entries) %s (%u entries)\n",
                      b->wgs_per_cu, b->lds_bytes, (size_t)(160 * 1024) / std::max<size_t>(b->lds_bytes, 1), n_l10,
                      a.l10_where == kL10Shared ? "in LDS" : a.l10_where == kL10Ring ? "through the ring" : "through L2", a.l10_lds_entries);
+    if (tm.on && b->mode == kMultiLds)
+        std::fprintf(stderr, "[svt] library windows: %u chunks, %d tiles per wave, tables as %s (rows over the largest window's bin space %zu B, its bins + descriptors %zu B)\n",
+                     b->n_chunks, b->window_tiles, b->binspace ? "shared bin space" : "descriptors", binspace_lds - kSBins, window_lds - kSBins);
     if (b->lds_bytes > 64 * 1024)
         for (int tiles = 1; tiles <= 2; ++tiles)
             if (b->mode != kGeneral || tiles == 1)
diff --git a/svtyper_amd/csrc/svt_batch_state.h b/svtyper_amd/csrc/svt_batch_state.h
--- a/svtyper_amd/csrc/svt_batch_state.h
+++ b/svtyper_amd/csrc/svt_batch_state.h
@@ -130,8 +130,16 @@
                      : reinterpret_cast<const void*>(&svt_stream_kernel<false, kMultiLds, 2, 2>);
 }
 
+template <bool SSO>
+const void* binspace_kernel_for(int tiles)
+{
+    return tiles == 2 ? reinterpret_cast<const void*>(&svt_stream_kernel<SSO, kMultiLds, 2, 3>)
+                      : reinterpret_cast<const void*>(&svt_stream_kernel<SSO, kMultiLds, SVT_STREAM_R, 3>);
+}
+
 const void* stream_kernel_of(const svt_batch* b, int tiles = SVT_STREAM_R)
 {
+    if (b->mode == kMultiLds && b->binspace) return (b->flags & SVT_FLAG_SSO_ASSOCIATION) ? binspace_kernel_for<true>(tiles) : binspace_kernel_for<false>(tiles);
     return (b->flags & SVT_FLAG_SSO_ASSOCIATION) ? stream_kernel_for<true>(b->mode, tiles) : stream_kernel_for<false>(b->mode, tiles);
 }
 
@@ -144,6 +152,10 @@
 const void* split_kernel_of(const svt_batch* b, int lanes)
 {
     const bool sso = (b->flags & SVT_FLAG_SSO_ASSOCIATION) != 0;
+    if (b->mode == kMultiLds && b->binspace) {
+        if (lanes == 2) return reinterpret_cast<const void*>(&svt_split_kernel<false, kMultiLds, 2, true>);
+        return sso ? reinterpret_cast<const void*>(&svt_split_kernel<true, kMultiLds, 4, true>) : reinterpret_cast<const void*>(&svt_split_kernel<false, kMultiLds, 4, true>);
+    }
     if (b->mode == kMultiLds) {
         if (lanes == 2) return reinterpret_cast<const void*>(&svt_split_kernel<false, kMultiLds, 2>);
         return sso ? reinterpret_cast<const void*>(&svt_split_kernel<true, kMultiLds, 4>) : reinterpret_cast<const void*>(&svt_split_kernel<false, kMultiLds, 4>);
diff --git a/svtyper_amd/csrc/svt_small_kernels.hip b/svtyper_amd/csrc/svt_small_kernels.hip
--- a/svtyper_amd/csrc/svt_small_kernels.hip
+++ b/svtyper_amd/csrc/svt_small_kernels.hip
@@ -15,6 +15,8 @@
 template __global__ void svt_stream_kernel<true, kSingleLds, 1>(const StreamArgs);
 template __global__ void svt_stream_kernel<false, kMultiLds, 1>(const StreamArgs);
 template __global__ void svt_stream_kernel<true, kMultiLds, 1>(const StreamArgs);
+template __global__ void svt_stream_kernel<false, kMultiLds, 1, 3>(const StreamArgs);
+template __global__ void svt_stream_kernel<true, kMultiLds, 1, 3>(const StreamArgs);
 template __global__ void svt_split_kernel<false, kSingleLds, 2>(const StreamArgs);
 template __global__ void svt_split_kernel<true, kSingleLds, 2>(const StreamArgs);
 template __global__ void svt_split_kernel<false, kSingleLds, 4>(const StreamArgs);
@@ -22,4 +24,7 @@
 template __global__ void svt_split_kernel<false, kMultiLds, 2>(const StreamArgs);
 template __global__ void svt_split_kernel<false, kMultiLds, 4>(const StreamArgs);
 template __global__ void svt_split_kernel<true, kMultiLds, 4>(const StreamArgs);
+template __global__ void svt_split_kernel<false, kMultiLds, 2, true>(const StreamArgs);
+template __global__ void svt_split_kernel<false, kMultiLds, 4, true>(const StreamArgs);
+template __global__ void svt_split_kernel<true, kMultiLds, 4, true>(const StreamArgs);
 }
diff --git a/svtyper_amd/csrc/svt_split_kernel.h b/svtyper_amd/csrc/svt_split_kernel.h
--- a/svtyper_amd/csrc/svt_split_kernel.h
+++ b/svtyper_amd/csrc/svt_split_kernel.h
@@ -56,9 +56,10 @@
     bool cont;
 };
 
-template <bool SSO, int MODE, int K>
+template <bool SSO, int MODE, int K, bool BINSPACE = false>
 __global__ __launch_bounds__(kBlock * K, 4) void svt_split_kernel(const StreamArgs a)
 {
+    static_assert(!BINSPACE || MODE == kMultiLds, "shared bin space: library windows only");
     static_assert(MODE == kSingleLds || MODE == kMultiLds, "one library, or library windows (svt_unit.libs)");
     static_assert(K == 2 || K == 4, "two or four lanes per unit");
     constexpr uint32_t kWaves = 4u * K, kThreads = kWaves * kWave, kUnitsPerWave = kWave / K, kRecs = kBlockRecords / K;
@@ -88,7 +89,7 @@
         cnt = (uint32_t)(hi - lo);
         U = a.units[my_unit];
     }
-    stage_tables<MODE, kThreads, false>(smem, a, wd, tid);
+    stage_tables<MODE, kThreads, false, BINSPACE>(smem, a, wd, tid);
     for (uint32_t i = tid; i < 5u * kBlock; i += kThreads) s_tally[i] = 0.0;
 
     {
@@ -127,7 +128,10 @@
             s_unit[pos] = my_unit;
             if (MODE == kMultiLds) {
                 uint32_t gated = 0u;
-                if (is_del)
+                if (is_del && BINSPACE)
+                    for (uint32_t l = 0; l < wd.lib_cnt; ++l)
+                        gated |= ((double)U.pos_delta < reinterpret_cast<const double*>(smem + a.lds_winlibs)[l] ? 1u : 0u) << l;
+                else if (is_del)
                     for (uint32_t l = 0; l < wd.lib_cnt; ++l)
                         gated |= ((double)U.pos_delta < reinterpret_cast<const WinLib*>(smem + a.lds_winlibs)[l].sd2 ? 1u : 0u) << l;
                 s_gate[pos] = gated;
@@ -161,6 +165,8 @@
     const uint32_t gated = MODE == kMultiLds ? s_gate[pos] : 0u;
     const bool is_del = (me.w & kTileDel16) != 0u;
     const uint32_t lib_last = wd.lib_cnt - 1u, winlibs_at = a.lds_winlibs;
+    const uint32_t bs_row = binspace_row_entries(wd.bin_cnt) * 2u, bs_hist_at = kSBins + wd.lib_cnt * bs_row;
+    const uint32_t bs_sub2 = is_del ? sc.sub2 + wd.bin_lo : 0x80000000u;
     const uint32_t neutral_w = MODE == kMultiLds ? wd.lib_lo << SVT_REC_LIB_SHIFT : 0u;
     const uint32_t lib_key = MODE == kMultiLds && wd.lib_cnt == 1u ? wd.lib_lo << SVT_REC_LIB_SHIFT : 0u;
 
@@ -226,7 +232,15 @@
                 wj[q].z = mine ? w[j].z : 0u;
                 wj[q].w = mine ? w[j].w : neutral_w;
                 check.see(wj[q], lib_key);
-                if (MODE == kMultiLds) {
+                if (MODE == kMultiLds && BINSPACE) {
+                    const uint32_t rel = SVT_REC_LIB(wj[q].w) - wd.lib_lo;
+                    check.window_lib(rel);
+                    const uint32_t l = min(rel, lib_last), row = __umul24(l, bs_row);
+                    f3[q] = ((gated >> l) & 1u) ? 0u : (wj[q].w & 7u);
+                    const uint32_t i1 = min(wj[q].x - wd.bin_lo, wd.bin_cnt), i2 = min(wj[q].x - bs_sub2, wd.bin_cnt);
+                    thr1[q] = lds_i16(kSBins + row + (i1 << 1));
+                    h2[q] = lds_u16(bs_hist_at + row + (i2 << 1));
+                } else if (MODE == kMultiLds) {
                     const uint32_t rel = SVT_REC_LIB(wj[q].w) - wd.lib_lo;
                     check.window_lib(rel);
                     const uint32_t l = min(rel, lib_last);
diff --git a/svtyper_amd/csrc/svt_stream_kernel.h b/svtyper_amd/csrc/svt_stream_kernel.h
--- a/svtyper_amd/csrc/svt_stream_kernel.h
+++ b/svtyper_amd/csrc/svt_stream_kernel.h
@@ -123,10 +123,35 @@
     a.ref_span += pp * lds_f64(wa + kSWref);
 }
 
+struct BinspaceCtx {
+    uint32_t lib_lo;
+    uint32_t lib_last;
+    uint32_t row_bytes;
+    uint32_t gated;
+};
+template <bool SSO, bool EDGE, bool CONT, class CHECK>
+__device__ __forceinline__ void record_binspace(const u32x4 w, const bool mine, const StreamCtx& c, const BinspaceCtx& b, Acc& a, CHECK& check)
+{
+    const double pp = record_weights<SSO, EDGE, CONT>(w, mine, a);
+    check.window_lib(EDGE && !mine ? 0u : SVT_REC_LIB(w.w) - b.lib_lo);
+    const uint32_t l = min(SVT_REC_LIB(w.w) - b.lib_lo, b.lib_last);
+    const uint32_t open = (uint32_t)__builtin_amdgcn_sbfe((int32_t)b.gated, l, 1u);
+    const uint32_t f3 = w.w & 7u & open;
+    const uint32_t row = __umul24(l, b.row_bytes);
+    const uint32_t i1 = min(w.x - c.kmin, c.nb), i2 = min(w.x - c.sub2, c.nb);
+    const int32_t thr1 = lds_i16(kSBins + row + (i1 << 1));
+    const uint32_t h2 = lds_u16(c.hist_at + row + (i2 << 1));
+    const bool p_conc = (int32_t)h2 <= thr1;
+    const uint32_t wa = (p_conc ? c.wt1 : c.wt0) | (f3 << 3);
+    a.alt_span += pp * lds_f64(wa);
+    a.ref_span += pp * lds_f64(wa + kSWref);
+}
+
 template <bool SSO, int MODE, int R, int WK = 0>
-__global__ __launch_bounds__(kBlock, MODE == kSingleLds ? SVT_STREAM_WAVES : MODE == kMultiLds ? (WK ? 4 : SVT_WINDOW_WAVES) : 2) void svt_stream_kernel(const StreamArgs a)
+__global__ __launch_bounds__(kBlock, MODE == kSingleLds ? SVT_STREAM_WAVES : MODE == kMultiLds ? (WK == 1 || WK == 2 ? 4 : SVT_WINDOW_WAVES) : 2) void svt_stream_kernel(const StreamArgs a)
 {
-    static_assert(WK == 0 || (MODE == kMultiLds && !SSO), "window kinds: classic library-window kernels only");
+    static_assert(WK == 0 || (MODE == kMultiLds && (!SSO || WK == 3)), "window kinds: classic library-window kernels only");
+    constexpr bool kBinspace = WK == 3;
     extern __shared__ __attribute__((aligned(16))) unsigned char smem[];
     constexpr uint32_t kUnitsPerWg = kBlock * R;
     if (MODE != kGeneral && (uint32_t)(size_t)(__attribute__((address_space(3))) unsigned char*)smem != 0u) __builtin_trap();
@@ -152,7 +177,7 @@
         }
     }
 
-    stage_tables<MODE, kBlock, true>(smem, a, wd, tid);
+    stage_tables<MODE, kBlock, true, kBinspace>(smem, a, wd, tid);
     uint4 info[R];
     wg_sort_into_tiles<R>(rings, beg, cnt, n_here, tid, lane, wave, info);
 
@@ -226,7 +251,14 @@
             sc.wt1 = sc.wt0 + 8u * 8u;
             sc.wh0 = kSWhi + c.del16 * 4u;
         }
-        if (MODE == kMultiLds) {
+        if (MODE == kMultiLds && kBinspace) {
+            const bool small_del = c.is_del && (c.pos_delta_d < reinterpret_cast<const double*>(smem + a.lds_winlibs)[0]);
+            sc.fmask = small_del ? 0u : 7u;
+            sc.kmin = wd.bin_lo;
+            sc.nb = wd.bin_cnt;
+            sc.sub2 = c.is_del ? (uint32_t)U.var_length + wd.bin_lo : 0x80000000u;
+            sc.hist_at = kSBins + wd.lib_cnt * binspace_row_entries(wd.bin_cnt) * 2u;
+        } else if (MODE == kMultiLds) {
             const WinLib w0 = reinterpret_cast<const WinLib*>(smem + a.lds_winlibs)[0];
             const bool small_del = c.is_del && (c.pos_delta_d < w0.sd2);
             sc.fmask = small_del ? 0u : 7u;
@@ -245,11 +277,21 @@
         wc.wh0 = sc.wh0;
         wc.is_del = c.is_del;
         wc.gated = 0u;
-        if (MODE == kMultiLds && c.is_del) {
+        if (MODE == kMultiLds && !kBinspace && c.is_del) {
             for (uint32_t l = 0; l < wd.lib_cnt; ++l)
                 wc.gated |= (c.pos_delta_d < reinterpret_cast<const WinLib*>(smem + a.lds_winlibs)[l].sd2 ? 1u : 0u) << l;
         }
         wc.gated = ~wc.gated;
+        BinspaceCtx bc;
+        bc.lib_lo = wd.lib_lo;
+        bc.lib_last = wd.lib_cnt - 1u;
+        bc.row_bytes = binspace_row_entries(wd.bin_cnt) * 2u;
+        bc.gated = 0u;
+        if (MODE == kMultiLds && kBinspace && c.is_del) {
+            for (uint32_t l = 0; l < wd.lib_cnt; ++l)
+                bc.gated |= (c.pos_delta_d < reinterpret_cast<const double*>(smem + a.lds_winlibs)[l] ? 1u : 0u) << l;
+        }
+        bc.gated = ~bc.gated;
         Acc acc = {0.0, 0.0, 0.0, 0.0, 0.0, 0.0, 0.0, 0.0};
 
         auto consume = [&](const u32x4 (&w)[8], const uint32_t k, auto edge, auto window_kind, auto continuations) {
@@ -270,6 +312,7 @@
                     record_single<SSO, EDGE, CONT>(wj, mine, sc, acc);
                 } else if (MODE == kMultiLds) {
                     if (KIND == 1) record_single<SSO, EDGE, CONT>(wj, mine, sc, acc);
+                    else if (kBinspace) record_binspace<SSO, EDGE, CONT>(wj, mine, sc, bc, acc, check);
                     else record_window<SSO, EDGE, CONT>(wj, mine, wc, acc, check);
                 } else {
                     const uint32_t wy = mine ? wj.y : 0u, wz = mine ? wj.z : 0u;
@@ -336,6 +379,7 @@
                         wj.w = mine ? wj.w : neutral_w;
                         check.see(wj, lib_key);
                         if (MODE == kSingleLds || WK == 1 || (WK == 0 && !SSO && wd.lib_cnt == 1u)) record_single<SSO, false, true>(wj, true, sc, acc);
+                        else if (kBinspace) record_binspace<SSO, false, true>(wj, true, sc, bc, acc, check);
                         else record_window<SSO, false, true>(wj, true, wc, acc, check);
                     }
                     refill();
diff --git a/svtyper_amd/csrc/svt_wg_parts.h b/svtyper_amd/csrc/svt_wg_parts.h
--- a/svtyper_amd/csrc/svt_wg_parts.h
+++ b/svtyper_amd/csrc/svt_wg_parts.h
@@ -2,6 +2,7 @@
 #define SVT_WG_PARTS_H
 
 #include "svt_ring_engine.h"
+#include "svt_window_binspace.h"
 
 namespace svt {
 
@@ -90,7 +91,7 @@
     return MODE == kMultiLds && a.perm ? a.perm[wg_base + local] : wg_base + local;
 }
 
-template <int MODE, uint32_t THREADS, bool HI>
+template <int MODE, uint32_t THREADS, bool HI, bool BINSPACE = false>
 __device__ __forceinline__ void stage_tables(unsigned char* smem, const StreamArgs& a, const WgDesc& wd, const uint32_t tid)
 {
     for (uint32_t i = tid; i < 256; i += THREADS) {
@@ -119,6 +120,19 @@
             s_thr[i] = (int16_t)bn.thr;
             s_hst[i] = (uint16_t)bn.hist;
         }
+    } else if (MODE == kMultiLds && BINSPACE) {
+        const uint32_t row = binspace_row_entries(wd.bin_cnt);
+        int16_t* s_thr = reinterpret_cast<int16_t*>(smem + kSBins);
+        uint16_t* s_hst = reinterpret_cast<uint16_t*>(smem + kSBins) + wd.lib_cnt * row;
+        for (uint32_t l = 0; l < wd.lib_cnt; ++l) {
+            const LibDesc L = a.libs[wd.lib_lo + l];
+            for (uint32_t j = tid; j < row; j += THREADS) {
+                const Bin bn = a.bins[L.tab_off + binspace_source_bin(j, (int32_t)wd.bin_lo, L.key_min, L.n_bins)];
+                s_thr[l * row + j] = (int16_t)bn.thr;
+                s_hst[l * row + j] = (uint16_t)bn.hist;
+            }
+        }
+        if (tid < wd.lib_cnt) reinterpret_cast<double*>(smem + a.lds_winlibs)[tid] = a.libs[wd.lib_lo + tid].sd2;
     } else if (MODE == kMultiLds) {
         int16_t* s_thr = reinterpret_cast<int16_t*>(smem + kSBins);
         uint16_t* s_hst = reinterpret_cast<uint16_t*>(smem + kSBins) + wd.bin_cnt;
diff --git a/svtyper_amd/csrc/svt_window_binspace.h b/svtyper_amd/csrc/svt_window_binspace.h
--- /dev/null
+++ b/svtyper_amd/csrc/svt_window_binspace.h
@@ -0,0 +1,50 @@
+#ifndef SVT_WINDOW_BINSPACE_H
+#define SVT_WINDOW_BINSPACE_H
+
+#include <stdint.h>
+
+#if defined(__HIP__)
+#define SVT_BS_HD __host__ __device__ inline __attribute__((always_inline))
+#else
+#define SVT_BS_HD inline
+#endif
+
+namespace svt {
+
+struct BinSpace {
+    int32_t k0;
+    uint32_t nb;
+};
+
+SVT_BS_HD BinSpace binspace_of(const int32_t* key_min, const uint32_t* n_bins, const uint32_t count, const uint32_t stride_words = 1u)
+{
+    int64_t lo = key_min[0], hi = (int64_t)key_min[0] + (int64_t)n_bins[0];
+    for (uint32_t l = 1; l < count; ++l) {
+        const int64_t k = key_min[(uint64_t)l * stride_words], e = k + (int64_t)n_bins[(uint64_t)l * stride_words];
+        lo = k < lo ? k : lo;
+        hi = e > hi ? e : hi;
+    }
+    BinSpace s;
+    s.k0 = (int32_t)lo;
+    s.nb = (uint32_t)(hi - lo);
+    return s;
+}
+
+SVT_BS_HD uint32_t binspace_source_bin(const uint32_t j, const int32_t k0, const int32_t key_min, const uint32_t n_bins)
+{
+    const uint32_t own = j + (uint32_t)k0 - (uint32_t)key_min;
+    return own < n_bins ? own : n_bins;
+}
+
+SVT_BS_HD uint32_t binspace_entry(const uint32_t span, const uint32_t sub, const uint32_t nb)
+{
+    const uint32_t j = span - sub;
+    return j < nb ? j : nb;
+}
+
+SVT_BS_HD uint32_t binspace_row_entries(const uint32_t nb) { return nb + 1u; }
+SVT_BS_HD uint64_t binspace_table_bytes(const uint32_t lib_cnt, const uint32_t nb) { return (uint64_t)lib_cnt * (nb + 1u) * 4u; }
+
+}
+
+#endif
diff --git a/svtyper_amd/csrc/svtyper_hip.hip b/svtyper_amd/csrc/svtyper_hip.hip
--- a/svtyper_amd/csrc/svtyper_hip.hip
+++ b/svtyper_amd/csrc/svtyper_hip.hip
@@ -54,6 +54,8 @@
 extern template __global__ void svt_stream_kernel<true, kSingleLds, 1>(const StreamArgs);
 extern template __global__ void svt_stream_kernel<false, kMultiLds, 1>(const StreamArgs);
 extern template __global__ void svt_stream_kernel<true, kMultiLds, 1>(const StreamArgs);
+extern template __global__ void svt_stream_kernel<false, kMultiLds, 1, 3>(const StreamArgs);
+extern template __global__ void svt_stream_kernel<true, kMultiLds, 1, 3>(const StreamArgs);
 extern template __global__ void svt_split_kernel<false, kSingleLds, 2>(const StreamArgs);
 extern template __global__ void svt_split_kernel<true, kSingleLds, 2>(const StreamArgs);
 extern template __global__ void svt_split_kernel<false, kSingleLds, 4>(const StreamArgs);
@@ -61,6 +63,9 @@
 extern template __global__ void svt_split_kernel<false, kMultiLds, 2>(const StreamArgs);
 extern template __global__ void svt_split_kernel<false, kMultiLds, 4>(const StreamArgs);
 extern template __global__ void svt_split_kernel<true, kMultiLds, 4>(const StreamArgs);
+extern template __global__ void svt_split_kernel<false, kMultiLds, 2, true>(const StreamArgs);
+extern template __global__ void svt_split_kernel<false, kMultiLds, 4, true>(const StreamArgs);
+extern template __global__ void svt_split_kernel<true, kMultiLds, 4, true>(const StreamArgs);
 }
 #endif
 
@@ -107,6 +112,7 @@
     uint32_t n_chunks = 0;
     uint32_t n_chunks_one = 0;
     bool split_window_kinds = false;
+    bool binspace = false;
     int window_tiles = 1;
     uint64_t bound_slots = 0;
     uint64_t out_slots = 0;
```

Result: slower. 3.185 billion (-7.5%).
